# itz-sayak/C-Users-Sayakdutta-Self-Supervised-Arbitrary-Scale-Point-Cloud-Upsampling-via-SNN

Hardware: AMD Instinct MI355X
Metric: upsampled query-points/sec (kNN + fn fwd + rotate + fd fwd + displace), 4x scale, M=48 T=4 (higher is better)
Workload: dtype f32 (GEMMs as 3 x f16 MFMA with f32 accumulation; outer kNN f64); 1 GPU; synthetic sphere N=5000 (seed 0), B=4096 grid queries per GPU per step, M=48, T=4, fn k=[24,18,12] emb 640, fd k=32 scales [8,16,32,48] emb 768, conditioned-random weights seed 0, in-patch kNN recomputed every batch; cloud_points=5000, neighbours=48, outer_knn=f64 brute force, parallelism=query shards x1

## Files before the change

### c-users-sayakdutta-self-supervised-arbitrary-scale-point-cloud-upsampling-via-snn_amd/csrc/fn_edge_chain.hip

```cpp
#include "common.h"
#include "gemm_epi.h"
#include "ops.h"

namespace sapcu {
typedef _Float16 half8 __attribute__((ext_vector_type(8)));

#ifndef SAPCU_CHAIN_LB128
#define SAPCU_CHAIN_LB128 3
#endif
template <int D> struct ChainShape {
    static constexpr int ROWS = D == 128 ? 96 : (D == 256 ? 128 : 64);
    static constexpr int RS = ROWS / 16;
    static constexpr int CB = D == 512 ? 2 : 1;
    static constexpr int CS = 2 * CB;
    static constexpr int NW = D / (32 * CB);
    static constexpr int PLANE = ROWS * 64;
    static constexpr int KSTEP = 2 * PLANE;
    static constexpr int LDS = ROWS * D * 4 + ROWS * 16 + ROWS * 8;
    static constexpr int US = 8;
};

template <int D, int KK> struct ChainSlots {
    static constexpr int GS = 4 * ChainShape<D>::RS;
    static constexpr int SP = GS - KK;
    static constexpr int NUA = (4 * SP) / KK;
    static constexpr int PPG = 4 + NUA;
    static constexpr int point(int rs, int g, int e) {
        const int t = 4 * rs + e;
        if (t < KK) return g;
        const int p = 4 + (g * SP + t - KK) / KK;
        return p < PPG ? p : -1;
    }
    static constexpr int nbr(int rs, int g, int e) {
        const int t = 4 * rs + e;
        return t < KK ? t : (g * SP + t - KK) % KK;
    }
    static constexpr int SP1 = SP > 0 ? SP : 1;
    static constexpr int ua_g(int n, int jj) { return (n * KK + jj) / SP1; }
    static constexpr int ua_rs(int n, int jj) { return (KK + (n * KK + jj) % SP1) >> 2; }
    static constexpr int ua_e(int n, int jj) { return (KK + (n * KK + jj) % SP1) & 3; }
};

__global__ __launch_bounds__(256) void edge_prep_kernel(const float* __restrict__ patch, const int32_t* __restrict__ idx,
                                                        int64_t rows, int m, int kk, int2* __restrict__ tab,
                                                        float4* __restrict__ pd) {
    const int64_t r = (int64_t)blockIdx.x * blockDim.x + threadIdx.x;
    if (r >= rows) return;
    const int64_t pt = r / kk;
    const int64_t nrow = (pt / m) * m + idx[r];
    tab[r] = make_int2((int)pt, (int)nrow);
    const float* pi = patch + pt * 3;
    const float* pj = patch + nrow * 3;
    pd[r] = make_float4(__fsub_rn(pi[0], pj[0]), __fsub_rn(pi[1], pj[1]), __fsub_rn(pi[2], pj[2]), 0.f);
}

__global__ __launch_bounds__(256) void pack_chain_weights_kernel(const _Float16* __restrict__ hi, const _Float16* __restrict__ lo,
                                                                 int d, _Float16* __restrict__ out) {
    const int64_t t = (int64_t)blockIdx.x * blockDim.x + threadIdx.x;
    const int nk32 = d / 32;
    const int64_t total = (int64_t)(d / 16) * nk32 * 2 * 64;
    if (t >= total) return;
    const int lane = (int)(t & 63);
    const int plane = (int)((t >> 6) & 1);
    const int64_t cs_s = t >> 7;
    const int s = (int)(cs_s % nk32), cs = (int)(cs_s / nk32);
    const _Float16* src = (plane ? lo : hi) + (int64_t)(16 * cs + (lane & 15)) * d + 32 * s + 8 * (lane >> 4);
    *reinterpret_cast<half8*>(out + t * 8) = *reinterpret_cast<const half8*>(src);
}

__device__ __forceinline__ float group_bcast(float x, int s) {
    const unsigned a = __float_as_uint(x);
    const auto r = __builtin_amdgcn_permlane16_swap(a, a, false, false);
    const unsigned z = (s & 1) ? r[1] : r[0];
    const auto q = __builtin_amdgcn_permlane32_swap(z, z, false, false);
    return __uint_as_float((s & 2) ? q[1] : q[0]);
}

template <int CS>
struct ChainLane {
    int c16, g;
    int col[CS];
    unsigned xw[CS];
};

template <int CS>
struct ChainW {
    half8 wh[CS], wl[CS];
};

template <int D>
__device__ __forceinline__ half8 chain_w_frag(const half8* __restrict__ wp, int cs, int s, int plane, int lane) {
    return wp[(((int64_t)cs * (D / 32) + s) * 2 + plane) * 64 + lane];
}

template <int D>
__device__ __forceinline__ void chain_w_prefetch(const half8* __restrict__ wp, int cs0, int lane, ChainW<ChainShape<D>::CS>& W) {
#pragma unroll
    for (int j = 0; j < ChainShape<D>::CS; ++j) {
        W.wh[j] = chain_w_frag<D>(wp, cs0 + j, 0, 0, lane);
        W.wl[j] = chain_w_frag<D>(wp, cs0 + j, 0, 1, lane);
    }
}

template <int D>
__device__ __forceinline__ void chain_gemm(const unsigned char* X, const half8* __restrict__ wp, int cs0, int lane,
                                           ChainW<ChainShape<D>::CS>& W, f32x4 (&acc)[ChainShape<D>::RS][ChainShape<D>::CS]) {
    constexpr int NK32 = D / 32, RS = ChainShape<D>::RS, CS = ChainShape<D>::CS, HC = CS / 2;
    constexpr int CH_PLANE = ChainShape<D>::PLANE, CH_KSTEP = ChainShape<D>::KSTEP;
    const int c16 = lane & 15, g = lane >> 4;
    const unsigned char* xa = X + c16 * 64 + ((g ^ ((c16 >> 2) & 3)) * 16);
#pragma unroll
    for (int i = 0; i < RS; ++i)
#pragma unroll
        for (int j = 0; j < CS; ++j) acc[i][j] = f32x4{0.f, 0.f, 0.f, 0.f};
    if (D == 128) {
        constexpr int RH = RS / 2;
#pragma unroll 1
        for (int s = 0; s < NK32; ++s) {
            const int sn = s + 1 < NK32 ? s + 1 : NK32 - 1;
#pragma unroll
            for (int rc = 0; rc < 2; ++rc) {
                half8 ah[RH], al[RH];
#pragma unroll
                for (int i = 0; i < RH; ++i) {
                    ah[i] = *reinterpret_cast<const half8*>(xa + s * CH_KSTEP + (rc * RH + i) * 1024);
                    al[i] = *reinterpret_cast<const half8*>(xa + s * CH_KSTEP + (rc * RH + i) * 1024 + CH_PLANE);
                }
#pragma unroll
                for (int hc = 0; hc < 2; ++hc) {
#pragma unroll
                    for (int i = 0; i < RH; ++i)
#pragma unroll
                        for (int j = hc * HC; j < (hc + 1) * HC; ++j)
                            acc[rc * RH + i][j] = __builtin_amdgcn_mfma_f32_16x16x32_f16(al[i], W.wh[j], acc[rc * RH + i][j], 0, 0, 0);
#pragma unroll
                    for (int i = 0; i < RH; ++i)
#pragma unroll
                        for (int j = hc * HC; j < (hc + 1) * HC; ++j)
                            acc[rc * RH + i][j] = __builtin_amdgcn_mfma_f32_16x16x32_f16(ah[i], W.wl[j], acc[rc * RH + i][j], 0, 0, 0);
#pragma unroll
                    for (int i = 0; i < RH; ++i)
#pragma unroll
                        for (int j = hc * HC; j < (hc + 1) * HC; ++j)
                            acc[rc * RH + i][j] = __builtin_amdgcn_mfma_f32_16x16x32_f16(ah[i], W.wh[j], acc[rc * RH + i][j], 0, 0, 0);
                    if (rc == 1) {
                        __builtin_amdgcn_sched_barrier(0);
#pragma unroll
                        for (int j = hc * HC; j < (hc + 1) * HC; ++j) {
                            W.wh[j] = chain_w_frag<D>(wp, cs0 + j, sn, 0, lane);
                            W.wl[j] = chain_w_frag<D>(wp, cs0 + j, sn, 1, lane);
                        }
                    }
                }
                __builtin_amdgcn_sched_barrier(0);
            }
        }
        return;
    }
#pragma unroll 1
    for (int s = 0; s < NK32; ++s) {
        half8 ah[RS], al[RS];
#pragma unroll
        for (int i = 0; i < RS; ++i) {
            ah[i] = *reinterpret_cast<const half8*>(xa + s * CH_KSTEP + i * 1024);
            al[i] = *reinterpret_cast<const half8*>(xa + s * CH_KSTEP + i * 1024 + CH_PLANE);
        }
        const int sn = s + 1 < NK32 ? s + 1 : NK32 - 1;
#pragma unroll
        for (int hc = 0; hc < 2; ++hc) {
#pragma unroll
            for (int i = 0; i < RS; ++i)
#pragma unroll
                for (int j = hc * HC; j < (hc + 1) * HC; ++j) acc[i][j] = __builtin_amdgcn_mfma_f32_16x16x32_f16(al[i], W.wh[j], acc[i][j], 0, 0, 0);
#pragma unroll
            for (int i = 0; i < RS; ++i)
#pragma unroll
                for (int j = hc * HC; j < (hc + 1) * HC; ++j) acc[i][j] = __builtin_amdgcn_mfma_f32_16x16x32_f16(ah[i], W.wl[j], acc[i][j], 0, 0, 0);
#pragma unroll
            for (int i = 0; i < RS; ++i)
#pragma unroll
                for (int j = hc * HC; j < (hc + 1) * HC; ++j) acc[i][j] = __builtin_amdgcn_mfma_f32_16x16x32_f16(ah[i], W.wh[j], acc[i][j], 0, 0, 0);
            __builtin_amdgcn_sched_barrier(0);
#pragma unroll
            for (int j = hc * HC; j < (hc + 1) * HC; ++j) {
                W.wh[j] = chain_w_frag<D>(wp, cs0 + j, sn, 0, lane);
                W.wl[j] = chain_w_frag<D>(wp, cs0 + j, sn, 1, lane);
            }
        }
    }
}

typedef _Float16 half2v __attribute__((ext_vector_type(2)));
template <int PLANE, int CS>
__device__ __forceinline__ void chain_put2(unsigned char* X, const ChainLane<CS>& L, int cs, int rs, int e, float v0, float v1) {
    unsigned char* p = X + L.xw[cs] + (unsigned)(rs * 1024 + e * 64);
    const f32x2 v = f32x2{v0, v1};
    const half2v hi = __builtin_convertvector(v, half2v);
    half2v lo;
    {
        unsigned lp;
        const unsigned hp = __builtin_bit_cast(unsigned, hi);
        asm volatile("v_fma_mixlo_f16 %0, %1, -1.0, %2 op_sel_hi:[1,0,0]" : "=v"(lp) : "v"(hp), "v"(v.x));
        asm volatile("v_fma_mixhi_f16 %0, %1, -1.0, %2 op_sel:[1,0,0] op_sel_hi:[1,0,0]" : "+v"(lp) : "v"(hp), "v"(v.y));
        lo = __builtin_bit_cast(half2v, lp);
    }
    *reinterpret_cast<_Float16*>(p) = hi.x;
    *reinterpret_cast<_Float16*>(p + 64) = hi.y;
    *reinterpret_cast<_Float16*>(p + PLANE) = lo.x;
    *reinterpret_cast<_Float16*>(p + PLANE + 64) = lo.y;
}

__device__ __forceinline__ void chain_store_split_nt(float* base, int64_t row, int ld, int col, float v) {
    _Float16* rp = reinterpret_cast<_Float16*>(base + row * ld);
    const _Float16 hi = (_Float16)v;
    __builtin_nontemporal_store(hi, &rp[split_hi_index(ld, col)]);
    __builtin_nontemporal_store((_Float16)(v - (float)hi), &rp[split_lo_index(ld, col)]);
}

__device__ __forceinline__ NeuronP chain_lif(const float* __restrict__ lif, int d, int col) {
    NeuronP np;
    np.decay = clampf(lif[col], 0.1f, 0.99f);
    np.adapt = clampf(lif[d + col], 0.001f, 0.1f);
    np.rdecay = clampf(lif[2 * d + col], 0.1f, 0.95f);
    np.theta0 = lif[3 * d + col];
    np.dT = 0.f;
    np.rh = 0.f;
    return np;
}

__device__ __forceinline__ float group_select(float v0, float v1, float v2, float v3, bool g0, bool g1) {
    const float a = g0 ? v1 : v0, b = g0 ? v3 : v2;
    return g1 ? b : a;
}

template <int KK>
__device__ __forceinline__ float chain_softmax_agg(float (&xs)[KK], const float (&ts)[KK]) {
    float mx = -__builtin_huge_valf();
#pragma unroll
    for (int jj = 0; jj < KK; ++jj) mx = fmaxf(mx, xs[jj]);
    float den = 0.f;
    const f32x2 mx2 = f32x2{mx, mx}, l2e = f32x2{1.4426950408889634074f, 1.4426950408889634074f};
#pragma unroll
    for (int jj = 0; jj < KK; jj += 2) {
        const f32x2 e2 = (f32x2{xs[jj], xs[jj + 1]} - mx2) * l2e;
        xs[jj] = __builtin_amdgcn_exp2f(e2.x);
        xs[jj + 1] = __builtin_amdgcn_exp2f(e2.y);
        den = __fadd_rn(den, xs[jj]);
        den = __fadd_rn(den, xs[jj + 1]);
    }
    const float inv_den = __fdiv_rn(1.0f, den);
    const f32x2 inv2 = f32x2{inv_den, inv_den};
    float out = 0.f;
#pragma unroll
    for (int jj = 0; jj < KK; jj += 2) {
        const f32x2 w2 = f32x2{xs[jj], xs[jj + 1]} * inv2;
        out = __fmaf_rn(w2.x, ts[jj], out);
        out = __fmaf_rn(w2.y, ts[jj + 1], out);
    }
    return out;
}

template <int D, int KK, bool O32, bool FILL>
__device__ __forceinline__ void fn_edge_chain_body(const ChainArgs& a) {
    static_assert(!FILL || (D == 512 && KK == 12), "filled groups: d = 512, kk = 12");
    using S = ChainShape<D>;
    using M = ChainSlots<D, KK>;
    constexpr int CH_ROWS = S::ROWS, RS = S::RS, CS = S::CS, CH_PLANE = S::PLANE, CH_KSTEP = S::KSTEP;
    constexpr int PPG = M::PPG, NUA = M::NUA, SP = M::SP;
    constexpr int NUP = RS / 2;
    extern __shared__ __attribute__((aligned(1024))) unsigned char smem[];
    unsigned char* X = smem;
    float* pdx = reinterpret_cast<float*>(smem + CH_ROWS * D * 4);
    float* pdy = pdx + CH_ROWS;
    float* pdz = pdy + CH_ROWS;
    int2* rinfo = reinterpret_cast<int2*>(smem + CH_ROWS * D * 4 + CH_ROWS * 16);

    const int tid = threadIdx.x;
    const int lane = tid & 63;
    const int w = __builtin_amdgcn_readfirstlane(tid >> 6);
    const int cs0 = w * CS;
    ChainLane<CS> L;
    L.c16 = lane & 15;
    L.g = lane >> 4;
    const bool g0 = (L.g & 1) != 0, g1 = (L.g & 2) != 0;
#pragma unroll
    for (int j = 0; j < CS; ++j) {
        L.col[j] = 16 * (cs0 + j) + L.c16;
        L.xw[j] = (unsigned)((L.col[j] >> 5) * CH_KSTEP + L.g * 256 + ((((L.col[j] >> 3) & 3) ^ L.g) * 16) + (L.col[j] & 7) * 2);
    }
    const int rowg = 4 * L.g;

    const int64_t nsuper = FILL ? a.P / 16 : 0;
    const int64_t ngroups = 3 * nsuper + (a.P - 16 * nsuper + PPG - 1) / PPG;
    int64_t grp;
    {
        const int64_t nx = gridDim.x < 8 ? 1 : 8;
        const int64_t x = nx == 1 ? 0 : (blockIdx.x & 7), slot = nx == 1 ? blockIdx.x : (blockIdx.x >> 3);
        const int64_t qd = ngroups / nx, rem = ngroups % nx;
        grp = x * qd + (x < rem ? x : rem) + slot;
        if (slot >= qd + (x < rem ? 1 : 0)) return;
    }
    int64_t pt0 = grp * PPG, strad = -1;
    int spos = 0;
    if (FILL) {
        if (grp < 3 * nsuper) {
            const unsigned sgi = (unsigned)grp / 3u;
            spos = (int)((unsigned)grp - 3u * sgi);
            pt0 = 16 * (int64_t)sgi + PPG * spos;
            strad = 16 * (int64_t)sgi + 15;
        } else {
            pt0 = 16 * nsuper + (grp - 3 * nsuper) * PPG;
        }
    }
    const int npts = (int)((a.P - pt0) < PPG ? (a.P - pt0) : PPG);

    f32x4 acc[RS][CS], pe[RS][CS];
    ChainW<CS> W;
    if (tid < CH_ROWS) {
        const int rs = tid >> 4, sg = (tid >> 2) & 3, e = tid & 3, t = 4 * rs + e;
        int p, jj;
        if (t < KK) {
            p = sg;
            jj = t;
        } else {
            const int u = sg * SP + t - KK;
            p = 4 + u / KK;
            jj = u % KK;
        }
        const bool ok = p < npts;
        int64_t er = ok ? (pt0 + p) * KK + jj : pt0 * KK;
        if (FILL && p >= PPG && strad >= 0) er = strad * KK + 4 * spos + jj;
        const int2 t2 = a.tab[er];
        if (O32) reinterpret_cast<unsigned*>(rinfo)[tid] = (unsigned)t2.y * (unsigned)(a.ldq * 4);
        else rinfo[tid] = t2;
        const float4 dv = a.pd[er];
        pdx[tid] = dv.x;
        pdy[tid] = dv.y;
        pdz[tid] = dv.z;
    }
    lds_barrier();
#pragma unroll
    for (int j = 0; j < CS; ++j) {
        const float wx = a.wd[L.col[j] * 3], wy = a.wd[L.col[j] * 3 + 1], wz = a.wd[L.col[j] * 3 + 2], bd = a.bd[L.col[j]];
        const NeuronP nd = chain_lif(a.lifd, D, L.col[j]);
#pragma unroll
        for (int up = 0; up < NUP; ++up) {
            float v[8];
#pragma unroll
            for (int hq = 0; hq < 2; ++hq) {
                const int r0 = 16 * (2 * up + hq) + rowg;
                const float4 qx = *reinterpret_cast<const float4*>(pdx + r0), qy = *reinterpret_cast<const float4*>(pdy + r0),
                             qz = *reinterpret_cast<const float4*>(pdz + r0);
                const f32x2 wx2 = f32x2{wx, wx}, wy2 = f32x2{wy, wy}, wz2 = f32x2{wz, wz}, bd2 = f32x2{bd, bd};
                const f32x2 ta = pk_fma(wz2, f32x2{qz.x, qz.y}, pk_fma(wy2, f32x2{qy.x, qy.y}, wx2 * f32x2{qx.x, qx.y})) + bd2;
                const f32x2 tb = pk_fma(wz2, f32x2{qz.z, qz.w}, pk_fma(wy2, f32x2{qy.z, qy.w}, wx2 * f32x2{qx.z, qx.w})) + bd2;
                v[4 * hq] = ta.x;
                v[4 * hq + 1] = ta.y;
                v[4 * hq + 2] = tb.x;
                v[4 * hq + 3] = tb.y;
            }
            lif_selfloop_n<8>(v, nd, a.T);
#pragma unroll
            for (int z = 0; z < 8; z += 2) chain_put2<CH_PLANE, CS>(X, L, j, 2 * up + (z >> 2), z & 3, v[z], v[z + 1]);
            __builtin_amdgcn_sched_barrier(0);
        }
    }
    const half8* const wp1 = reinterpret_cast<const half8*>(a.w1p);
    const half8* const wp2 = reinterpret_cast<const half8*>(a.w2p);
    const half8* const wp3 = reinterpret_cast<const half8*>(a.w3p);
    float kq[2][8], vq[2][8];
    auto gather_kv = [&](int j, int up, float (&kd)[8], float (&vd)[8]) {
#pragma unroll
        for (int z = 0; z < 8; ++z) {
            const int row = 16 * (2 * up + (z >> 2)) + rowg + (z & 3);
            if (O32) {
                const unsigned off = reinterpret_cast<const unsigned*>(rinfo)[row] + 4u * (unsigned)L.col[j];
                kd[z] = *reinterpret_cast<const float*>(reinterpret_cast<const char*>(a.qkv + D) + off);
                vd[z] = *reinterpret_cast<const float*>(reinterpret_cast<const char*>(a.qkv + 2 * D) + off);
            } else {
                const int nrow = rinfo[row].y;
                kd[z] = a.qkv[(int64_t)nrow * a.ldq + D + L.col[j]];
                vd[z] = a.qkv[(int64_t)nrow * a.ldq + 2 * D + L.col[j]];
            }
        }
    };
    auto load_q = [&](int j, float& qa, float (&qu)[NUA > 0 ? NUA : 1], float& qs) {
        qa = __builtin_nontemporal_load(&a.qkv[(pt0 + (L.g < npts ? L.g : 0)) * a.ldq + L.col[j]]);
        if (FILL) qs = __builtin_nontemporal_load(&a.qkv[(strad >= 0 ? strad : pt0) * a.ldq + L.col[j]]);
#pragma unroll
        for (int n = 0; n < NUA; ++n) qu[n] = __builtin_nontemporal_load(&a.qkv[(pt0 + (4 + n < npts ? 4 + n : 0)) * a.ldq + L.col[j]]);
    };
    float qa[2], qu[2][NUA > 0 ? NUA : 1], qs[2] = {0.f, 0.f};
    load_q(0, qa[0], qu[0], qs[0]);
    gather_kv(0, 0, kq[0], vq[0]);
    chain_w_prefetch<D>(wp1, cs0, lane, W);
    lds_barrier();

    {
        chain_gemm<D>(X, wp1, cs0, lane, W, acc);
        lds_barrier();
#pragma unroll
        for (int j = 0; j < CS; ++j) {
            const float b1 = a.b1[L.col[j]];
            const NeuronP n1 = chain_lif(a.lif1, D, L.col[j]);
            if (j + 1 < CS) load_q(j + 1, qa[(j + 1) & 1], qu[(j + 1) & 1], qs[(j + 1) & 1]);
#pragma unroll
            for (int up = 0; up < NUP; ++up) {
                const int u = j * NUP + up;
                if (up + 1 < NUP) gather_kv(j, up + 1, kq[(u + 1) & 1], vq[(u + 1) & 1]);
                else if (j + 1 < CS) gather_kv(j + 1, 0, kq[(u + 1) & 1], vq[(u + 1) & 1]);
                __builtin_amdgcn_sched_barrier(0);
                float v[8];
#pragma unroll
                for (int z = 0; z < 8; ++z) v[z] = __fmaf_rn(acc[2 * up + (z >> 2)][j][z & 3], 0.0625f, b1);
                lif_selfloop_n<8>(v, n1, a.T);
                __builtin_amdgcn_sched_barrier(0);
                float ain[8];
#pragma unroll
                for (int z = 0; z < 8; ++z) {
                    const int rs = 2 * up + (z >> 2), e = z & 3;
                    float qv;
                    if (4 * rs + e < KK) {
                        qv = qa[j & 1];
                    } else {
                        float c[4];
#pragma unroll
                        for (int sg = 0; sg < 4; ++sg) {
                            const int p = M::point(rs, sg, e);
                            c[sg] = p >= 4 ? qu[j & 1][p - 4 < NUA ? p - 4 : 0] : (FILL && p < 0 ? qs[j & 1] : qa[j & 1]);
                        }
                        qv = group_select(c[0], c[1], c[2], c[3], g0, g1);
                    }
                    ain[z] = __fadd_rn(__fsub_rn(qv, kq[u & 1][z]), v[z]);
                    pe[rs][j][e] = settle(__fadd_rn(vq[u & 1][z], v[z]));
                }
#pragma unroll
                for (int z = 0; z < 8; z += 2) chain_put2<CH_PLANE, CS>(X, L, j, 2 * up + (z >> 2), z & 3, ain[z], ain[z + 1]);
                __builtin_amdgcn_sched_barrier(0);
            }
        }
        chain_w_prefetch<D>(wp2, cs0, lane, W);
    }
    lds_barrier();
    {
        chain_gemm<D>(X, wp2, cs0, lane, W, acc);
        lds_barrier();
#pragma unroll
        for (int j = 0; j < CS; ++j) {
            const float b2 = a.b2[L.col[j]];
            const NeuronP n2 = chain_lif(a.lif2, D, L.col[j]);
#pragma unroll
            for (int up = 0; up < NUP; ++up) {
                float v[8];
#pragma unroll
                for (int z = 0; z < 8; ++z) v[z] = __fmaf_rn(acc[2 * up + (z >> 2)][j][z & 3], 0.0625f, b2);
                lif_selfloop_n<8>(v, n2, a.T);
#pragma unroll
                for (int z = 0; z < 8; z += 2) chain_put2<CH_PLANE, CS>(X, L, j, 2 * up + (z >> 2), z & 3, v[z], v[z + 1]);
                __builtin_amdgcn_sched_barrier(0);
            }
        }
        chain_w_prefetch<D>(wp3, cs0, lane, W);
    }
    lds_barrier();
    {
        chain_gemm<D>(X, wp3, cs0, lane, W, acc);
#pragma unroll
        for (int j = 0; j < CS; ++j) {
            const float b3 = a.b3[L.col[j]];
#pragma unroll
            for (int i = 0; i < RS; ++i) {
                const f32x2 k16 = f32x2{0.0625f, 0.0625f}, b32 = f32x2{b3, b3}, is2 = f32x2{a.inv_sqrt_hd, a.inv_sqrt_hd};
                const f32x2 lo = pk_fma(f32x2{acc[i][j][0], acc[i][j][1]}, k16, b32) * is2;
                const f32x2 hi = pk_fma(f32x2{acc[i][j][2], acc[i][j][3]}, k16, b32) * is2;
                acc[i][j] = f32x4{lo.x, lo.y, hi.x, hi.y};
            }
            if (FILL) {
                if (L.g == 3 && strad >= 0) {
                    const int64_t o = ((strad >> 4) * KK + 4 * spos) * D + L.col[j];
#pragma unroll
                    for (int e = 0; e < 4; ++e) {
                        __builtin_nontemporal_store(acc[RS - 1][j][e], &a.fill_x[o + e * D]);
                        __builtin_nontemporal_store(pe[RS - 1][j][e], &a.fill_t[o + e * D]);
                    }
                }
            }
            {
                float xs[KK], ts[KK];
#pragma unroll
                for (int jj = 0; jj < KK; ++jj) {
                    xs[jj] = acc[jj >> 2][j][jj & 3];
                    ts[jj] = pe[jj >> 2][j][jj & 3];
                }
                const float out = chain_softmax_agg<KK>(xs, ts);
                if (L.g < npts) {
                    const int64_t pt = pt0 + L.g;
                    if (a.res_split) chain_store_split_nt(a.res, pt, D, L.col[j], out);
                    else __builtin_nontemporal_store(out, &a.res[pt * D + L.col[j]]);
                }
            }
            if (NUA > 0) {
                float xs[KK], ts[KK];
#pragma unroll
                for (int jj = 0; jj < KK; ++jj) {
                    float cx[4] = {0.f, 0.f, 0.f, 0.f}, ct[4] = {0.f, 0.f, 0.f, 0.f};
#pragma unroll
                    for (int n = 0; n < NUA; ++n) {
                        const int rs = M::ua_rs(n, jj), e = M::ua_e(n, jj), sg = M::ua_g(n, jj);
                        cx[n] = group_bcast(acc[rs][j][e], sg);
                        ct[n] = group_bcast(pe[rs][j][e], sg);
                    }
                    xs[jj] = NUA == 1 ? cx[0] : group_select(cx[0], cx[1], cx[2], cx[3], g0, g1);
                    ts[jj] = NUA == 1 ? ct[0] : group_select(ct[0], ct[1], ct[2], ct[3], g0, g1);
                }
                const float out = chain_softmax_agg<KK>(xs, ts);
                if (L.g < NUA && 4 + L.g < npts) {
                    const int64_t pt = pt0 + 4 + L.g;
                    if (a.res_split) chain_store_split_nt(a.res, pt, D, L.col[j], out);
                    else __builtin_nontemporal_store(out, &a.res[pt * D + L.col[j]]);
                }
            }
        }
    }
}

template <int D, int KK, bool O32>
__global__ __launch_bounds__(ChainShape<D>::NW * 64, (D == 128 ? SAPCU_CHAIN_LB128 : 1)) void fn_edge_chain_kernel(const ChainArgs a) {
    fn_edge_chain_body<D, KK, O32, false>(a);
}

template <bool O32>
__global__ __launch_bounds__(ChainShape<512>::NW * 64, 1) void fn_edge_chain_fill_kernel(const ChainArgs a) {
    fn_edge_chain_body<512, 12, O32, true>(a);
}

template <int KK>
__global__ __launch_bounds__(256) void fn_chain_straddler_kernel(const float* __restrict__ fx, const float* __restrict__ ft, int64_t nsuper,
                                                                 int d, float* __restrict__ res, int res_split) {
    const int64_t t = (int64_t)blockIdx.x * blockDim.x + threadIdx.x;
    if (t >= nsuper * d) return;
    const int64_t sgi = t / d;
    const int col = (int)(t - sgi * d);
    float xs[KK], ts[KK];
#pragma unroll
    for (int jj = 0; jj < KK; ++jj) {
        xs[jj] = __builtin_nontemporal_load(&fx[(sgi * KK + jj) * d + col]);
        ts[jj] = __builtin_nontemporal_load(&ft[(sgi * KK + jj) * d + col]);
    }
    const float out = chain_softmax_agg<KK>(xs, ts);
    const int64_t pt = 16 * sgi + 15;
    if (res_split) chain_store_split_nt(res, pt, d, col, out);
    else __builtin_nontemporal_store(out, &res[pt * d + col]);
}

template <int D, int KK, bool O32>
static int launch_chain_t(const ChainArgs& a, hipStream_t st) {
    constexpr int lds = ChainShape<D>::LDS;
    static DeviceOnce lds_once;
    SAPCU_SET_MAX_LDS(lds_once, (&fn_edge_chain_kernel<D, KK, O32>), lds);
    constexpr int PPG = ChainSlots<D, KK>::PPG;
    const int64_t ngroups = (a.P + PPG - 1) / PPG;
    const int64_t grid = ngroups < 8 ? ngroups : ((ngroups + 7) / 8) * 8;
    SAPCU_CHECK_ARG(grid < 0x7fffffffLL, "edge_chain: too many groups");
    hipLaunchKernelGGL((fn_edge_chain_kernel<D, KK, O32>), dim3((unsigned)grid), dim3(ChainShape<D>::NW * 64), lds, st, a);
    SAPCU_CHECK_LAUNCH();
    return SAPCU_OK;
}

template <bool O32>
static int launch_chain_fill_t(const ChainArgs& a, hipStream_t st) {
    constexpr int lds = ChainShape<512>::LDS, PPG = ChainSlots<512, 12>::PPG;
    static DeviceOnce lds_once;
    SAPCU_SET_MAX_LDS(lds_once, (&fn_edge_chain_fill_kernel<O32>), lds);
    const int64_t nsuper = a.P / 16;
    const int64_t ngroups = 3 * nsuper + (a.P - 16 * nsuper + PPG - 1) / PPG;
    const int64_t grid = ngroups < 8 ? ngroups : ((ngroups + 7) / 8) * 8;
    SAPCU_CHECK_ARG(grid < 0x7fffffffLL, "edge_chain: too many groups");
    hipLaunchKernelGGL((fn_edge_chain_fill_kernel<O32>), dim3((unsigned)grid), dim3(ChainShape<512>::NW * 64), lds, st, a);
    SAPCU_CHECK_LAUNCH();
    hipLaunchKernelGGL((fn_chain_straddler_kernel<12>), dim3((unsigned)((nsuper * 512 + 255) / 256)), dim3(256), 0, st, a.fill_x, a.fill_t,
                       nsuper, 512, a.res, a.res_split);
    SAPCU_CHECK_LAUNCH();
    return SAPCU_OK;
}

bool fn_edge_chain_ok(int d, int kk) { return (d == 128 && kk == 24) || (d == 256 && kk == 18) || (d == 512 && kk == 12); }

int launch_fn_edge_chain(ChainArgs a, const float* patch, const int32_t* idx, int d, int kk, int2* tab, float4* pd,
                         hipStream_t st) {
    if (a.P == 0) return SAPCU_OK;
    SAPCU_CHECK_ARG(fn_edge_chain_ok(d, kk), "edge_chain: unsupported block shape d=%d kk=%d", d, kk);
    SAPCU_CHECK_ARG(a.P * (int64_t)kk < 0x7fffffffLL && a.P * (int64_t)(a.ldq) < (1LL << 40), "edge_chain: too many rows");
    const int64_t rows = a.P * kk;
    hipLaunchKernelGGL(edge_prep_kernel, dim3((unsigned)((rows + 255) / 256)), dim3(256), 0, st, patch, idx, rows, a.m, kk, tab, pd);
    SAPCU_CHECK_LAUNCH();
    a.tab = tab;
    a.pd = pd;
    const bool o32 = !a.wide_offsets && (uint64_t)a.P * (uint64_t)a.ldq * 4u + 3u * (uint64_t)d * 4u < (1ull << 32) && a.ldq > 0;
    if (d == 128) return o32 ? launch_chain_t<128, 24, true>(a, st) : launch_chain_t<128, 24, false>(a, st);
    if (d == 256) return o32 ? launch_chain_t<256, 18, true>(a, st) : launch_chain_t<256, 18, false>(a, st);
    if (a.fill_x && a.fill_t && a.P >= 16) return o32 ? launch_chain_fill_t<true>(a, st) : launch_chain_fill_t<false>(a, st);
    return o32 ? launch_chain_t<512, 12, true>(a, st) : launch_chain_t<512, 12, false>(a, st);
}

int launch_pack_chain_weights(const void* w16_hi, const void* w16_lo, int d, void* out, hipStream_t st) {
    const int64_t total = (int64_t)(d / 16) * (d / 32) * 2 * 64;
    hipLaunchKernelGGL(pack_chain_weights_kernel, dim3((unsigned)((total + 255) / 256)), dim3(256), 0, st,
                       (const _Float16*)w16_hi, (const _Float16*)w16_lo, d, (_Float16*)out);
    SAPCU_CHECK_LAUNCH();
    return SAPCU_OK;
}

}
```

### c-users-sayakdutta-self-supervised-arbitrary-scale-point-cloud-upsampling-via-snn_amd/csrc/model.hip

```cpp
#include <stdarg.h>
#include <stdlib.h>

#include <new>
#include <vector>

#include "common.h"
#include "ops.h"

namespace sapcu {

static thread_local char g_err[512] = "";

void set_error(const char* fmt, ...) {
    va_list ap;
    va_start(ap, fmt);
    vsnprintf(g_err, sizeof(g_err), fmt, ap);
    va_end(ap);
}

enum FnSlot {
    FN_STEM_W = 0, FN_STEM_B, FN_STEM_LIF,
    FN_BLK0 = 3,
    FN_FINAL_W = FN_BLK0 + 63, FN_FINAL_B, FN_FINAL_LIF,
    FN_FCOUT_W, FN_FCOUT_B,
    FN_MLP0_W, FN_MLP0_B, FN_MLP1_W, FN_MLP1_B, FN_MLP2_W, FN_MLP2_B,
    FN_HEAD_W, FN_HEAD_B, FN_LN_W, FN_LN_B,
    FN_SLOTS
};
enum FnBlkSlot {
    B_FC1_W = 0, B_FC1_B, B_SNN1,
    B_QKV_W, B_QKV_B, B_QKV_LIF,
    B_DELTA_W, B_DELTA_B, B_DELTA_LIF,
    B_DELTA2_W, B_DELTA2_B, B_DELTA2_LIF,
    B_GAMMA_W, B_GAMMA_B, B_GAMMA_LIF,
    B_GAMMA2_W, B_GAMMA2_B,
    B_OUT_W, B_OUT_B,
    B_FC2_W, B_FC2_B,
    B_SLOTS
};
static_assert(B_SLOTS == 21, "fn block slot count");
static_assert(FN_SLOTS == 81, "fn slot count");

enum FdSlot {
    FD_E0_W = 0, FD_E0_B,
    FD_FUSE_W, FD_FUSE_B, FD_SNN0,
    FD_EDGE1_W, FD_EDGE1_SHIFT, FD_SNN1,
    FD_EDGE2_W, FD_EDGE2_SHIFT, FD_SNN2,
    FD_EDGE3_W, FD_EDGE3_SHIFT, FD_SNN3,
    FD_MSC_W, FD_MSC_B,
    FD_TI_W, FD_SNNFC,
    FD_FCIN_W, FD_FCIN_B,
    FD_R0_FC0_W, FD_R0_FC0_B, FD_R0_FC4_W, FD_R0_FC4_B, FD_R0_PROJ_W, FD_R0_PROJ_B,
    FD_R1_FC0_W, FD_R1_FC0_B, FD_R1_FC4_W, FD_R1_FC4_B, FD_R1_PROJ_W, FD_R1_PROJ_B,
    FD_QKV_W, FD_QKV_B,
    FD_WO_T, FD_BO, FD_LN_W, FD_LN_B, FD_WH_T, FD_BH, FD_WD, FD_BD,
    FD_SLOTS
};
static_assert(FD_SLOTS == 42, "fd slot count");

}

struct sapcu_model {
    int kind = 0;
    int kv[3] = {0, 0, 0};
    int k = 0, nscale = 0;
    int ks[8] = {0, 0, 0, 0, 0, 0, 0, 0};
    int32_t* ks_dev = nullptr;
    int* gate_dev = nullptr;
    bool sf16 = true;
    void* w16_hi = nullptr;
    void* w16_lo = nullptr;
    void* chain_w = nullptr;
    int* ovf_dev = nullptr;
    int emb = 0, T = 0, heads = 0;
    int64_t chunk = 0;
    int64_t ws_budget = 0;
    bool opt_bt = true;
    bool opt_chain = true;
    bool opt_chain_wide = false;
    bool opt_chain_fill = true;
    bool opt_shortk = true;
    bool opt_fn_maxfuse = true;
    bool opt_fn_fold_out = true;
    bool opt_fd_maxfuse = true;
    bool opt_fd_split = true;
    bool opt_fd_fused = true;
    bool opt_fd_x0 = true;
    void* fde_w = nullptr;
    int64_t fde_off[5] = {0, 0, 0, 0, 0};
    float* fde_nprm = nullptr;
    float* blob = nullptr;
    int64_t blob_floats = 0;
    int64_t fold_w[3] = {0, 0, 0}, fold_b[3] = {0, 0, 0};
    std::vector<int64_t> dir;
    const float* p(int slot) const { return blob + dir[slot]; }
};

namespace sapcu {

static inline int64_t imax(int64_t a, int64_t b) { return a > b ? a : b; }
static inline int imin(int a, int b) { return a < b ? a : b; }

static bool split_rows_gemm_on_big_tile(const GemmArgs& g, bool allow_bt) { return allow_bt && gemm_sf16_bt_ok(g); }

int launch_gemm_split_rows(const GemmArgs& g, hipStream_t st, bool allow_bt) {
    if (split_rows_gemm_on_big_tile(g, allow_bt)) return launch_gemm_sf16_bt(g, st);
    return launch_gemm_sf16_ring(g, st);
}

static void fold_affine_f64(const float* w1, const float* b1, const float* w2, const float* b2, int d, int n, float* w_fold,
                            float* b_fold) {
    std::vector<double> acc((size_t)d);
    for (int i = 0; i < n; ++i) {
        for (int k = 0; k < d; ++k) acc[k] = 0.0;
        double bs = 0.0;
        for (int j = 0; j < d; ++j) {
            const double a = (double)w2[(int64_t)i * d + j];
            const float* row = w1 + (int64_t)j * d;
            for (int k = 0; k < d; ++k) acc[k] += a * (double)row[k];
            bs += a * (double)b1[j];
        }
        for (int k = 0; k < d; ++k) w_fold[(int64_t)i * d + k] = (float)acc[k];
        b_fold[i] = (float)(bs + (double)b2[i]);
    }
}

static bool env_is(const char* name, const char* value) {
    const char* e = getenv(name);
    return e && strcmp(e, value) == 0;
}

static void read_env_switches(sapcu_model* m) {
    m->sf16 = !env_is("SAPCU_GEMM", "f32");
    m->opt_bt = !env_is("SAPCU_BT", "0");
    m->opt_chain = !env_is("SAPCU_CHAIN", "0");
    m->opt_chain_wide = env_is("SAPCU_CHAIN", "wide");
    m->opt_chain_fill = !env_is("SAPCU_CHAIN_FILL", "0");
    m->opt_shortk = !env_is("SAPCU_SHORTK", "0");
    m->opt_fn_maxfuse = !env_is("SAPCU_FN_MAXFUSE", "0");
    m->opt_fn_fold_out = !env_is("SAPCU_FN_FOLD_OUT", "0");
    m->opt_fd_maxfuse = !env_is("SAPCU_FD_MAXFUSE", "0");
    m->opt_fd_split = !env_is("SAPCU_FD_SPLIT", "0");
    m->opt_fd_fused = !env_is("SAPCU_FD_FUSED", "0");
    m->opt_fd_x0 = !env_is("SAPCU_FD_X0", "0");
    const char* ce = getenv("SAPCU_CHUNK");
    m->chunk = ce ? atoll(ce) : 0;
    if (m->chunk < 0) m->chunk = 0;
    const char* be = getenv("SAPCU_WS_BUDGET_MB");
    m->ws_budget = (be ? atoll(be) : 20480) * (int64_t)(1 << 20);
    if (m->ws_budget < (int64_t)(64 << 20)) m->ws_budget = (int64_t)(64 << 20);
}

static void free_model(sapcu_model* m) {
    void* const owned[] = {m->w16_hi, m->w16_lo, m->chain_w, m->ovf_dev, m->blob, m->ks_dev, m->gate_dev, m->fde_w, m->fde_nprm};
    for (void* p : owned)
        if (p) (void)hipFree(p);
    delete m;
}

static int run_gemm(const sapcu_model* m, GemmArgs& g, hipStream_t st) {
    const bool have16 = m && m->sf16 && g.w >= m->blob && g.w < m->blob + m->blob_floats;
    if (have16) {
        const int64_t off = g.w - m->blob;
        g.w16_hi = (const _Float16*)m->w16_hi + off;
        g.w16_lo = (const _Float16*)m->w16_lo + off;
        g.ovf = m->ovf_dev;
        if (g.a_split) return launch_gemm_split_rows(g, st, m->opt_bt);
        if (m->opt_shortk && gemm_shortk_ok(g)) return launch_gemm_shortk(g, st);
        if (g.max_out) {
            set_error("run_gemm: a direct max output needs the short-K kernel");
            return SAPCU_ERR_ARG;
        }
        if (g.k % 64 == 0) return launch_gemm_sf16(g, st);
    }
    if (g.a_split || g.c_split || g.c2_split) {
        set_error("run_gemm: split-row operands need the split-f16 kernels");
        return SAPCU_ERR_ARG;
    }
    return launch_gemm(g, st);
}

static int gemm(const sapcu_model* m, const float* a, int64_t r, int k, int lda, const float* w, int n,
                const float* bias, float* c, int ldc, int epi, hipStream_t st, const float* lif = nullptr,
                int lifT = 0, const float* resid = nullptr, int ldr = 0, int fmt = 0) {
    GemmArgs g;
    memset(&g, 0, sizeof(g));
    g.a = a; g.r = r; g.k = k; g.lda = lda; g.w = w; g.n = n; g.bias = bias; g.c = c; g.ldc = ldc;
    g.epi = epi; g.lif = lif; g.lif_T = lifT; g.resid = resid; g.ldr = ldr;
    g.a_split = fmt & 1; g.c_split = (fmt >> 1) & 1;
    return run_gemm(m, g, st);
}

#define SAPCU_TRY(expr)                 \
    do {                                \
        int _rc = (expr);               \
        if (_rc != SAPCU_OK) return _rc; \
    } while (0)

static int tap_copy(void* const* taps, int which, int64_t dst_off_bytes, const void* src, int64_t bytes,
                    hipStream_t st) {
    if (!taps || !taps[which] || bytes == 0) return SAPCU_OK;
    SAPCU_CHECK_HIP(hipMemcpyAsync((char*)taps[which] + dst_off_bytes, src, (size_t)bytes, hipMemcpyDeviceToDevice, st));
    return SAPCU_OK;
}

struct FnPlan {
    int64_t cb;
    int kk[3], kmx;
    int64_t edge_floats, edge_floats23;
};

static bool fn_block_fused(const sapcu_model* m, int l, int mp) {
    return m->sf16 && m->chain_w && m->opt_chain && fn_edge_chain_ok(128 << l, imin(m->kv[l], mp));
}

static int fn_kmax(const sapcu_model* m, int mp) {
    int kmx = 1;
    for (int l = 0; l < 3; ++l) kmx = kmx > imin(m->kv[l], mp) ? kmx : imin(m->kv[l], mp);
    return kmx;
}

static void fn_edge_floats_per_patch(const sapcu_model* m, int mp, int64_t& first, int64_t& others) {
    first = (int64_t)mp * m->emb;
    others = 0;
    for (int l = 0; l < 3; ++l) {
        if (fn_block_fused(m, l, mp)) continue;
        const int64_t e = (int64_t)mp * imin(m->kv[l], mp) * (128 << l);
        first = imax(first, e);
        others = imax(others, e);
    }
}

static int64_t fn_bytes_per_patch(const sapcu_model* m, int mp) {
    int64_t e1, e23;
    fn_edge_floats_per_patch(m, mp, e1, e23);
    int64_t idxs = 0;
    for (int l = 0; l < 3; ++l) idxs += (int64_t)mp * imin(m->kv[l], mp) * 4;
    return (e1 + 2 * e23) * 4 + idxs + (int64_t)mp * fn_kmax(m, mp) * 24 + (int64_t)mp * (64 + 192 + 512 + 1536 + 512) * 4 +
           ((int64_t)m->emb + 2048 + 1024 + 512 + 256 + 3) * 4;
}

static int64_t chunk_patches(const sapcu_model* m, int64_t b, int64_t bytes_per_patch) {
    int64_t cb = m->chunk;
    if (cb <= 0) {
        cb = m->ws_budget / (bytes_per_patch > 0 ? bytes_per_patch : 1);
        cb = cb < 64 ? 64 : (cb / 64) * 64;
    }
    if (cb > b) cb = b;
    return cb < 1 ? 1 : cb;
}

static FnPlan fn_plan(const sapcu_model* m, int64_t b, int mp) {
    FnPlan pl;
    pl.cb = chunk_patches(m, b, fn_bytes_per_patch(m, mp));
    for (int l = 0; l < 3; ++l) pl.kk[l] = imin(m->kv[l], mp);
    pl.kmx = fn_kmax(m, mp);
    int64_t e1, e23;
    fn_edge_floats_per_patch(m, mp, e1, e23);
    pl.edge_floats = e1 * pl.cb;
    pl.edge_floats23 = e23 * pl.cb;
    return pl;
}

struct FnWs {
    int32_t* idx[3];
    int2* tab;
    float4* pdiff;
    float *feat0, *cat, *X, *QKV, *RES;
    float* B1;
    float *B2, *B3;
    float *pooled, *enc, *h1, *h2, *h3, *logits;
    size_t bytes;
};

static FnWs fn_ws_layout(void* base, const sapcu_model* m, const FnPlan& pl, int mp) {
    const int64_t P = pl.cb * mp;
    WsCarver c(base);
    FnWs w;
    for (int l = 0; l < 3; ++l) w.idx[l] = c.take<int32_t>(P * pl.kk[l]);
    w.tab = c.take<int2>(P * pl.kmx);
    w.pdiff = c.take<float4>(P * pl.kmx);
    w.feat0 = c.take<float>(P * 64);
    w.cat = c.take<float>(P * 192);
    w.X = c.take<float>(P * 512);
    w.QKV = c.take<float>(P * 1536);
    w.RES = c.take<float>(P * 512);
    w.B1 = c.take<float>(pl.edge_floats);
    w.B2 = c.take<float>(pl.edge_floats23);
    w.B3 = c.take<float>(pl.edge_floats23);
    w.pooled = c.take<float>(pl.cb * m->emb);
    w.enc = c.take<float>(pl.cb * 2048);
    w.h1 = c.take<float>(pl.cb * 1024);
    w.h2 = c.take<float>(pl.cb * 512);
    w.h3 = c.take<float>(pl.cb * 256);
    w.logits = c.take<float>(pl.cb * 3);
    w.bytes = c.bytes();
    return w;
}

static int64_t chain_w_off(int l, int q) {
    int64_t off = 0;
    for (int i = 0; i < l; ++i) off += (int64_t)3 * 2 * (128 << i) * (128 << i);
    return off + (int64_t)q * 2 * (128 << l) * (128 << l);
}

struct FnEdge {
    const float* pc;
    int64_t P;
    int mp, l, d, kk, sb, SP;
    float sqrt_hd;
    int64_t b1_floats;
};

static int fn_edge_chain_fused(const sapcu_model* m, const FnWs& W, const FnEdge& e, hipStream_t st) {
    const int d = e.d, sb = e.sb;
    ChainArgs ca;
    memset(&ca, 0, sizeof(ca));
    ca.P = e.P; ca.m = e.mp; ca.qkv = W.QKV; ca.ldq = 3 * d;
    ca.wd = m->p(sb + B_DELTA_W); ca.bd = m->p(sb + B_DELTA_B); ca.lifd = m->p(sb + B_DELTA_LIF);
    const _Float16* cw = (const _Float16*)m->chain_w;
    ca.w1p = cw + chain_w_off(e.l, 0); ca.b1 = m->p(sb + B_DELTA2_B); ca.lif1 = m->p(sb + B_DELTA2_LIF);
    ca.w2p = cw + chain_w_off(e.l, 1); ca.b2 = m->p(sb + B_GAMMA_B); ca.lif2 = m->p(sb + B_GAMMA_LIF);
    ca.w3p = cw + chain_w_off(e.l, 2); ca.b3 = m->p(sb + B_GAMMA2_B);
    ca.inv_sqrt_hd = 1.0f / e.sqrt_hd;
    ca.res = W.RES; ca.res_split = e.SP; ca.T = 4; ca.wide_offsets = m->opt_chain_wide ? 1 : 0;
    if (m->opt_chain_fill && d == 512 && e.kk == 12) {
        const int64_t need = (e.P / 16) * 12 * 512;
        if (need > 0 && need <= e.P * 512 && need <= e.b1_floats) {
            ca.fill_x = W.X;
            ca.fill_t = W.B1;
        }
    }
    return launch_fn_edge_chain(ca, e.pc, W.idx[e.l], d, e.kk, W.tab, W.pdiff, st);
}

static int fn_edge_chain_unfused(const sapcu_model* m, const FnWs& W, const FnEdge& e, hipStream_t st) {
    const int d = e.d, kk = e.kk, sb = e.sb, SP = e.SP;
    const int64_t R = e.P * kk;
    const int32_t* idx = W.idx[e.l];
    SAPCU_TRY(launch_fn_pe1(e.pc, idx, R, e.mp, kk, d, m->p(sb + B_DELTA_W), m->p(sb + B_DELTA_B), m->p(sb + B_DELTA_LIF), 4, W.B1, SP,
                            st));
    {
        GemmArgs g;
        memset(&g, 0, sizeof(g));
        g.a = W.B1; g.r = R; g.k = d; g.lda = d; g.w = m->p(sb + B_DELTA2_W); g.n = d;
        g.bias = m->p(sb + B_DELTA2_B); g.c = W.B2; g.ldc = d; g.epi = EPI_LIF_ATTN;
        g.lif = m->p(sb + B_DELTA2_LIF); g.lif_T = 4; g.c2 = W.B3;
        g.q = W.QKV; g.kf = W.QKV + d; g.ldq = 3 * d; g.tab = W.tab;
        g.a_split = SP; g.c2_split = SP;
        SAPCU_TRY(launch_edge_table(idx, R, e.mp, kk, W.tab, st));
        SAPCU_TRY(run_gemm(m, g, st));
    }
    SAPCU_TRY(gemm(m, W.B3, R, d, d, m->p(sb + B_GAMMA_W), d, m->p(sb + B_GAMMA_B), W.B1, d, EPI_LIF, st, m->p(sb + B_GAMMA_LIF), 4,
                   nullptr, 0, SP | (SP << 1)));
    SAPCU_TRY(gemm(m, W.B1, R, d, d, m->p(sb + B_GAMMA2_W), d, m->p(sb + B_GAMMA2_B), W.B3, d, EPI_BIAS, st, nullptr, 0, nullptr, 0, SP));
    return launch_fn_softmax_agg(W.B3, W.B2, W.QKV + 2 * d, 3 * d, idx, e.P, e.mp, kk, d, e.sqrt_hd, W.RES, SP, st);
}

static int fn_forward(const sapcu_model* m, const float* patch, int64_t b, int mp, const int32_t* knn_in,
                      int32_t* knn_out, float* normals, void* ws, int64_t ws_bytes, void* const* taps,
                      hipStream_t st) {
    const FnPlan pl = fn_plan(m, b, mp);
    const FnWs W = fn_ws_layout(ws_align256(ws), m, pl, mp);
    if (ws_bytes < (int64_t)W.bytes + 256) {
        set_error("fn_forward: workspace %lld B < required %lld B", (long long)ws_bytes, (long long)W.bytes + 256);
        return SAPCU_ERR_WORKSPACE;
    }
    int64_t tab_off[3];
    tab_off[0] = 0;
    tab_off[1] = b * mp * pl.kk[0];
    tab_off[2] = tab_off[1] + b * mp * pl.kk[1];

    for (int64_t s = 0; s < b; s += pl.cb) {
        const int64_t cb = (b - s) < pl.cb ? (b - s) : pl.cb;
        const int64_t P = cb * mp;
        const float* pc = patch + s * mp * 3;

        if (!knn_in) SAPCU_TRY(launch_patch_knn_multi(pc, cb, (int64_t)mp * 3, mp, 3, 3, 3, pl.kk, W.idx, st));
        for (int l = 0; l < 3; ++l) {
            const int64_t cnt = P * pl.kk[l];
            if (knn_in)
                SAPCU_CHECK_HIP(hipMemcpyAsync(W.idx[l], knn_in + tab_off[l] + s * mp * pl.kk[l], cnt * 4,
                                               hipMemcpyDeviceToDevice, st));
            if (knn_out)
                SAPCU_CHECK_HIP(hipMemcpyAsync(knn_out + tab_off[l] + s * mp * pl.kk[l], W.idx[l], cnt * 4,
                                               hipMemcpyDeviceToDevice, st));
        }
        SAPCU_TRY(launch_fn_stem(pc, P, m->p(FN_STEM_W), m->p(FN_STEM_B), m->p(FN_STEM_LIF), m->T, W.feat0, st));
        SAPCU_TRY(tap_copy(taps, SAPCU_FN_TAP_STEM, s * mp * 64 * 4, W.feat0, P * 64 * 4, st));

        const float* fin = W.feat0;
        int ldin = 64;
        for (int l = 0; l < 3; ++l) {
            const int d = 128 << l;
            const int sb = FN_BLK0 + l * B_SLOTS;
            const int SP = m->sf16 ? 1 : 0;
            float* const out = W.cat + 64 * l;
            SAPCU_TRY(gemm(m, fin, P, 64, ldin, m->p(sb + B_FC1_W), d, m->p(sb + B_FC1_B), W.X, d, EPI_LIF, st,
                           m->p(sb + B_SNN1), 4, nullptr, 0, SP << 1));
            SAPCU_TRY(gemm(m, W.X, P, d, d, m->p(sb + B_QKV_W), 3 * d, m->p(sb + B_QKV_B), W.QKV, 3 * d, EPI_LIF, st,
                           m->p(sb + B_QKV_LIF), 4, nullptr, 0, SP));
            const FnEdge e{pc, P, mp, l, d, pl.kk[l], sb, SP, (float)sqrt((double)(d / m->heads)), pl.edge_floats};
            SAPCU_TRY(fn_block_fused(m, l, mp) ? fn_edge_chain_fused(m, W, e, st) : fn_edge_chain_unfused(m, W, e, st));
            if (m->opt_fn_fold_out) {
                SAPCU_TRY(gemm(m, W.RES, P, d, d, m->blob + m->fold_w[l], 64, m->blob + m->fold_b[l], out, 192, EPI_RESID, st,
                               nullptr, 0, fin, ldin, SP));
            } else {
                SAPCU_TRY(gemm(m, W.RES, P, d, d, m->p(sb + B_OUT_W), d, m->p(sb + B_OUT_B), W.X, d, EPI_BIAS, st, nullptr, 0, nullptr,
                               0, SP | (SP << 1)));
                SAPCU_TRY(gemm(m, W.X, P, d, d, m->p(sb + B_FC2_W), 64, m->p(sb + B_FC2_B), out, 192, EPI_RESID, st,
                               nullptr, 0, fin, ldin, SP));
            }
            if (taps && taps[SAPCU_FN_TAP_BLOCK1 + l]) {
                SAPCU_CHECK_HIP(hipMemcpy2DAsync((char*)taps[SAPCU_FN_TAP_BLOCK1 + l] + s * mp * 64 * 4, 64 * 4,
                                                 out, 192 * 4, 64 * 4, (size_t)P, hipMemcpyDeviceToDevice, st));
            }
            fin = out;
            ldin = 192;
        }
        if (m->sf16 && m->opt_fn_maxfuse) {
            GemmArgs g;
            memset(&g, 0, sizeof(g));
            g.a = W.cat; g.r = P; g.k = 192; g.lda = 192; g.w = m->p(FN_FINAL_W); g.n = m->emb; g.bias = m->p(FN_FINAL_B);
            g.ldc = m->emb; g.epi = EPI_LIF_MAX; g.lif = m->p(FN_FINAL_LIF); g.lif_T = m->T;
            g.max_keys = reinterpret_cast<unsigned*>(W.B1); g.max_m = mp;
            const bool direct = m->opt_shortk && mp == 48;
            if (direct) g.max_out = W.pooled;
            else SAPCU_CHECK_HIP(hipMemsetAsync(g.max_keys, 0, (size_t)cb * m->emb * 4, st));
            SAPCU_TRY(run_gemm(m, g, st));
            if (!direct) SAPCU_TRY(launch_decode_max_keys(g.max_keys, cb * m->emb, W.pooled, st));
        } else {
            SAPCU_TRY(gemm(m, W.cat, P, 192, 192, m->p(FN_FINAL_W), m->emb, m->p(FN_FINAL_B), W.B1, m->emb, EPI_LIF, st,
                           m->p(FN_FINAL_LIF), m->T));
            SAPCU_TRY(launch_rowgroup_max(W.B1, cb, mp, m->emb, W.pooled, st));
        }
        SAPCU_TRY(tap_copy(taps, SAPCU_FN_TAP_POOLED, s * m->emb * 4, W.pooled, cb * m->emb * 4, st));
        SAPCU_TRY(gemm(m, W.pooled, cb, m->emb, m->emb, m->p(FN_FCOUT_W), 2048, m->p(FN_FCOUT_B), W.enc, 2048, EPI_BIAS, st));
        SAPCU_TRY(tap_copy(taps, SAPCU_FN_TAP_ENC, s * 2048 * 4, W.enc, cb * 2048 * 4, st));
        SAPCU_TRY(gemm(m, W.enc, cb, 2048, 2048, m->p(FN_MLP0_W), 1024, m->p(FN_MLP0_B), W.h1, 1024, EPI_GELU, st));
        SAPCU_TRY(gemm(m, W.h1, cb, 1024, 1024, m->p(FN_MLP1_W), 512, m->p(FN_MLP1_B), W.h2, 512, EPI_GELU, st));
        SAPCU_TRY(gemm(m, W.h2, cb, 512, 512, m->p(FN_MLP2_W), 256, m->p(FN_MLP2_B), W.h3, 256, EPI_GELU, st));
        SAPCU_TRY(launch_fn_tail(W.h3, cb, 256, m->p(FN_HEAD_W), m->p(FN_HEAD_B), m->p(FN_LN_W), m->p(FN_LN_B), W.logits,
                                 normals + s * 3, st));
        SAPCU_TRY(tap_copy(taps, SAPCU_FN_TAP_LOGITS, s * 3 * 4, W.logits, cb * 3 * 4, st));
    }
    return SAPCU_OK;
}

struct FdPlan {
    int64_t cb;
    int kmax0, kk;
    bool fused;
    bool x0path;
    bool maxfuse;
    int64_t agg_rows(int mp) const { return maxfuse ? 1 : mp; }
};

static bool fd_encoder_fused(const sapcu_model* m, int mp) {
    return m->sf16 && m->opt_fd_fused && m->fde_w && m->fde_nprm && fd_encoder_ok(mp, m->nscale, m->emb, m->T);
}

static bool fd_x0_path(const sapcu_model* m, int mp) {
    return !fd_encoder_fused(m, mp) && m->sf16 && m->opt_fd_fused && m->opt_fd_x0 && m->opt_fd_maxfuse && m->opt_fd_split && m->fde_w &&
           m->fde_nprm && fd_msc_ok(mp, m->emb, m->T);
}

static int fd_kmax0(const sapcu_model* m, int mp) {
    int kmax = 1;
    for (int i = 0; i < m->nscale; ++i) kmax = kmax > m->ks[i] ? kmax : m->ks[i];
    return imin(kmax, mp);
}

static FdPlan fd_plan(const sapcu_model* m, int64_t b, int mp) {
    FdPlan pl;
    pl.fused = fd_encoder_fused(m, mp);
    pl.x0path = fd_x0_path(m, mp);
    pl.maxfuse = m->sf16 && m->opt_fd_maxfuse;
    pl.kmax0 = fd_kmax0(m, mp);
    pl.kk = imin(m->k, mp);
    int64_t per_patch = ((int64_t)(m->T + 1) * m->emb + 256 + 3 * 128 + 3 * 64 + 192 + 64) * 4;
    if (!pl.fused) {
        const int64_t slabs = pl.x0path ? 2 : m->T;
        per_patch = (int64_t)mp * ((slabs * 960 + 960 + 1024 + 64 * (m->nscale + 1)) * 4 + (int64_t)(pl.kmax0 + 3 * pl.kk) * 4) +
                    (int64_t)m->T * pl.agg_rows(mp) * m->emb * 4 + per_patch;
    }
    pl.cb = chunk_patches(m, b, per_patch);
    return pl;
}

struct FdWs {
    int32_t* idx0;
    int32_t* idxb;
    float* E0;
    float* FUSED;
    float* SPK;
    float* F0;
    float* AB;
    float* AGG;
    float* X0;
    float *POOLED, *ENC;
    float *D1, *D2a, *D2b, *D2c, *D3a, *D3b, *D3c, *QKV, *ATT;
    size_t bytes;
};

static FdWs fd_ws_layout(void* base, const sapcu_model* m, const FdPlan& pl, int mp) {
    const int64_t cb = pl.cb, T = m->T, emb = m->emb;
    const int64_t P = pl.fused ? 0 : cb * mp;
    WsCarver c(base);
    FdWs w;
    w.idx0 = c.take<int32_t>(P * pl.kmax0);
    w.idxb = c.take<int32_t>(3 * P * pl.kk);
    w.E0 = c.take<float>(P * 64 * m->nscale);
    w.FUSED = c.take<float>(P * 64);
    w.SPK = c.take<float>((pl.x0path ? 1 : T) * P * 960);
    w.F0 = c.take<float>(P * 960);
    w.AB = c.take<float>(P * 1024);
    w.AGG = c.take<float>(pl.fused ? 0 : T * cb * pl.agg_rows(mp) * emb);
    w.X0 = c.take<float>(pl.x0path ? P * 960 : 0);
    w.POOLED = c.take<float>(T * cb * emb);
    w.ENC = c.take<float>(cb * emb);
    w.D1 = c.take<float>(cb * 256);
    w.D2a = c.take<float>(cb * 128);
    w.D2b = c.take<float>(cb * 128);
    w.D2c = c.take<float>(cb * 128);
    w.D3a = c.take<float>(cb * 64);
    w.D3b = c.take<float>(cb * 64);
    w.D3c = c.take<float>(cb * 64);
    w.QKV = c.take<float>(cb * 192);
    w.ATT = c.take<float>(cb * 64);
    w.bytes = c.bytes();
    return w;
}

struct FdChunk {
    const float* pc;
    int64_t s, cb, b;
    int mp;
    const int32_t* knn_force;
    void* const* taps;
    int64_t P() const { return cb * mp; }
    float* tap(int which) const { return taps ? (float*)taps[which] : nullptr; }
    float* x0_tap() const { return tap(SAPCU_FD_TAP_X0) ? tap(SAPCU_FD_TAP_X0) + s * mp * 960 : nullptr; }
};

static const int FD_CIN[4] = {0, 64, 128, 256}, FD_COUT[4] = {64, 128, 256, 512}, FD_COFF[4] = {0, 64, 192, 448};

static int fd_encode_fused(const sapcu_model* m, const FdPlan& pl, const FdWs& W, const FdChunk& c, hipStream_t st) {
    FdEncArgs ea;
    memset(&ea, 0, sizeof(ea));
    ea.patch = c.pc; ea.b = c.cb; ea.b_total = c.b; ea.s0 = c.s;
    ea.m = c.mp; ea.T = m->T; ea.kk = pl.kk; ea.kmax0 = pl.kmax0; ea.nscale = m->nscale; ea.emb = m->emb;
    for (int i = 0; i < 4; ++i) ea.ks[i] = i < m->nscale ? imin(m->ks[i], c.mp) : 0;
    ea.e0_w = m->p(FD_E0_W); ea.e0_b = m->p(FD_E0_B);
    const _Float16* fw = (const _Float16*)m->fde_w;
    ea.fuse_wp = fw + m->fde_off[0]; ea.fuse_b = m->p(FD_FUSE_B);
    for (int l = 0; l < 3; ++l) {
        ea.edge_wp[l] = fw + m->fde_off[1 + l];
        ea.shift[l] = m->p(FD_EDGE1_SHIFT + 3 * l);
    }
    ea.msc_wp = fw + m->fde_off[4]; ea.msc_b = m->p(FD_MSC_B);
    ea.nprm = m->fde_nprm;
    ea.pooled = W.POOLED;
    ea.knn_force = c.knn_force;
    ea.tap_knn = (int32_t*)c.tap(SAPCU_FD_TAP_KNN);
    ea.tap_fused0 = c.tap(SAPCU_FD_TAP_FUSED0);
    ea.tap_spikes = c.tap(SAPCU_FD_TAP_SPIKES);
    ea.tap_x0 = c.tap(SAPCU_FD_TAP_X0);
    ea.gate = m->gate_dev; ea.ovf = m->ovf_dev;
    return launch_fd_encoder(ea, st);
}

static GemmArgs fd_msc_gemm_args(const sapcu_model* m, const FdWs& W, const FdChunk& c) {
    GemmArgs mg;
    memset(&mg, 0, sizeof(mg));
    mg.a = W.SPK; mg.r = (int64_t)m->T * c.P(); mg.k = 960; mg.lda = 960; mg.w = m->p(FD_MSC_W); mg.n = m->emb; mg.bias = m->p(FD_MSC_B);
    mg.c = nullptr; mg.ldc = m->emb; mg.epi = EPI_LRELU_MAX; mg.max_keys = reinterpret_cast<unsigned*>(W.AGG); mg.max_m = c.mp;
    return mg;
}

static int fd_front(const sapcu_model* m, const FdPlan& pl, const FdWs& W, const FdChunk& c, bool& split_spikes, hipStream_t st) {
    const int T = m->T, mp = c.mp;
    const int64_t P = c.P(), cb = c.cb, s = c.s, b = c.b;
    void* const* taps = c.taps;
    SAPCU_TRY(launch_patch_knn(c.pc, cb, mp, 3, 3, pl.kmax0, W.idx0, st));
    SAPCU_TRY(launch_fd_edge0(c.pc, W.idx0, pl.kmax0, P, mp, m->nscale, m->ks_dev, m->p(FD_E0_W), m->p(FD_E0_B), W.E0, st));
    SAPCU_TRY(gemm(m, W.E0, P, 64 * m->nscale, 64 * m->nscale, m->p(FD_FUSE_W), 64, m->p(FD_FUSE_B), W.FUSED, 64, EPI_LRELU, st));
    SAPCU_TRY(tap_copy(taps, SAPCU_FD_TAP_FUSED0, s * mp * 64 * 4, W.FUSED, P * 64 * 4, st));
    float* const X0T = c.x0_tap();
    if (X0T) SAPCU_CHECK_HIP(hipMemcpy2DAsync(X0T, 960 * 4, W.FUSED, 64 * 4, 64 * 4, (size_t)P, hipMemcpyDeviceToDevice, st));
    split_spikes = pl.x0path;
    if (!pl.x0path && pl.maxfuse && m->opt_fd_split && !c.tap(SAPCU_FD_TAP_SPIKES)) {
        GemmArgs probe = fd_msc_gemm_args(m, W, c);
        probe.a_split = 1;
        probe.w16_hi = (const _Float16*)m->w16_hi + (probe.w - m->blob);
        probe.w16_lo = (const _Float16*)m->w16_lo + (probe.w - m->blob);
        split_spikes = split_rows_gemm_on_big_tile(probe, m->opt_bt);
    }
    float* const SPKS = split_spikes ? W.SPK : nullptr;
    float* const SPK0 = split_spikes ? W.F0 : W.SPK;
    float* const X0P = pl.x0path ? W.X0 : nullptr;
    SAPCU_TRY(launch_fd_neuron(true, 0, W.FUSED, 64, nullptr, 0, mp, nullptr, P, 64, m->p(FD_SNN0), T, SPK0, 960, 0,
                               nullptr, m->gate_dev, st, SPKS, X0P));
    for (int l = 1; l <= 3; ++l) {
        const int cin = FD_CIN[l], cout = FD_COUT[l], coff = FD_COFF[l - 1];
        int32_t* idl = W.idxb + (int64_t)(l - 1) * pl.cb * mp * pl.kk;
        const float* F = SPK0 + coff;
        if (c.knn_force) {
            SAPCU_CHECK_HIP(hipMemcpyAsync(idl, c.knn_force + ((int64_t)(l - 1) * b + s) * mp * pl.kk, P * pl.kk * 4,
                                           hipMemcpyDeviceToDevice, st));
        } else {
            SAPCU_TRY(launch_patch_knn_strided(F, cb, (int64_t)mp * 960, mp, cin, 960, pl.kk, idl, st));
        }
        if (c.tap(SAPCU_FD_TAP_KNN))
            SAPCU_CHECK_HIP(hipMemcpyAsync((int32_t*)taps[SAPCU_FD_TAP_KNN] + ((int64_t)(l - 1) * b + s) * mp * pl.kk,
                                           idl, P * pl.kk * 4, hipMemcpyDeviceToDevice, st));
        const int ew = FD_EDGE1_W + 3 * (l - 1);
        if (split_spikes)
            SAPCU_TRY(gemm(m, SPKS + coff, P, cin, 960, m->p(ew), 2 * cout, nullptr, W.AB, 2 * cout, EPI_BIAS, st, nullptr, 0, nullptr, 0,
                           1));
        else
            SAPCU_TRY(gemm(m, F, P, cin, 960, m->p(ew), 2 * cout, nullptr, W.AB, 2 * cout, EPI_BIAS, st));
        SAPCU_TRY(launch_fd_neuron(l == 1, 1, W.AB, 2 * cout, idl, pl.kk, mp, m->p(ew + 1), P, cout, m->p(ew + 2), T, SPK0, 960,
                                   FD_COFF[l], nullptr, m->gate_dev, st, SPKS, X0P));
        if (X0T && !pl.x0path)
            SAPCU_TRY(launch_fd_pre(W.AB, 2 * cout, idl, pl.kk, mp, m->p(ew + 1), P, cout, X0T, 960, FD_COFF[l], st));
    }
    return SAPCU_OK;
}

static int fd_msc_from_x0(const sapcu_model* m, const FdWs& W, const FdChunk& c, hipStream_t st) {
    if (c.x0_tap()) SAPCU_CHECK_HIP(hipMemcpyAsync(c.x0_tap(), W.X0, (size_t)c.P() * 960 * 4, hipMemcpyDeviceToDevice, st));
    FdMscArgs ma;
    memset(&ma, 0, sizeof(ma));
    ma.x0 = W.X0; ma.b = c.cb; ma.b_total = c.b; ma.s0 = c.s; ma.m = c.mp; ma.T = m->T; ma.emb = m->emb;
    ma.msc_wp = (const _Float16*)m->fde_w + m->fde_off[4]; ma.msc_b = m->p(FD_MSC_B); ma.nprm = m->fde_nprm;
    ma.pooled = W.POOLED; ma.tap_spikes = c.tap(SAPCU_FD_TAP_SPIKES); ma.gate = m->gate_dev;
    return launch_fd_msc(ma, st);
}

static int fd_msc_from_slabs(const sapcu_model* m, const FdPlan& pl, const FdWs& W, const FdChunk& c, bool split_spikes, hipStream_t st) {
    const int T = m->T, emb = m->emb;
    const int64_t P = c.P();
    if (c.tap(SAPCU_FD_TAP_SPIKES)) {
        for (int t = 0; t < T; ++t)
            SAPCU_CHECK_HIP(hipMemcpyAsync(c.tap(SAPCU_FD_TAP_SPIKES) + ((int64_t)t * c.b + c.s) * c.mp * 960,
                                           W.SPK + (int64_t)t * P * 960, P * 960 * 4, hipMemcpyDeviceToDevice, st));
    }
    if (pl.maxfuse) {
        GemmArgs mg = fd_msc_gemm_args(m, W, c);
        SAPCU_CHECK_HIP(hipMemsetAsync(mg.max_keys, 0, (size_t)T * c.cb * emb * 4, st));
        mg.a_split = split_spikes ? 1 : 0;
        SAPCU_TRY(run_gemm(m, mg, st));
        return launch_decode_max_keys(mg.max_keys, (int64_t)T * c.cb * emb, W.POOLED, st);
    }
    SAPCU_TRY(gemm(m, W.SPK, (int64_t)T * P, 960, 960, m->p(FD_MSC_W), emb, m->p(FD_MSC_B), W.AGG, emb, EPI_LRELU, st));
    return launch_rowgroup_max(W.AGG, (int64_t)T * c.cb, c.mp, emb, W.POOLED, st);
}

static int fd_temporal_decoder(const sapcu_model* m, const FdWs& W, const FdChunk& c, float* dist, hipStream_t st) {
    const int T = m->T, emb = m->emb;
    const int64_t cb = c.cb, s = c.s;
    if (c.tap(SAPCU_FD_TAP_POOLED)) {
        for (int t = 0; t < T; ++t)
            SAPCU_CHECK_HIP(hipMemcpyAsync(c.tap(SAPCU_FD_TAP_POOLED) + ((int64_t)t * c.b + s) * emb, W.POOLED + (int64_t)t * cb * emb,
                                           cb * emb * 4, hipMemcpyDeviceToDevice, st));
    }
    SAPCU_TRY(launch_fd_temporal(W.POOLED, T, cb, emb, m->p(FD_TI_W), m->p(FD_SNNFC), W.ENC, st));
    SAPCU_TRY(tap_copy(c.taps, SAPCU_FD_TAP_ENC, s * emb * 4, W.ENC, cb * emb * 4, st));
    SAPCU_TRY(gemm(m, W.ENC, cb, emb, emb, m->p(FD_FCIN_W), 256, m->p(FD_FCIN_B), W.D1, 256, EPI_GELU, st));
    SAPCU_TRY(gemm(m, W.D1, cb, 256, 256, m->p(FD_R0_FC0_W), 128, m->p(FD_R0_FC0_B), W.D2a, 128, EPI_GELU, st));
    SAPCU_TRY(gemm(m, W.D1, cb, 256, 256, m->p(FD_R0_PROJ_W), 128, m->p(FD_R0_PROJ_B), W.D2b, 128, EPI_BIAS, st));
    SAPCU_TRY(gemm(m, W.D2a, cb, 128, 128, m->p(FD_R0_FC4_W), 128, m->p(FD_R0_FC4_B), W.D2c, 128, EPI_RESID_GELU, st, nullptr, 0, W.D2b,
                   128));
    SAPCU_TRY(gemm(m, W.D2c, cb, 128, 128, m->p(FD_R1_FC0_W), 64, m->p(FD_R1_FC0_B), W.D3a, 64, EPI_GELU, st));
    SAPCU_TRY(gemm(m, W.D2c, cb, 128, 128, m->p(FD_R1_PROJ_W), 64, m->p(FD_R1_PROJ_B), W.D3b, 64, EPI_BIAS, st));
    SAPCU_TRY(gemm(m, W.D3a, cb, 64, 64, m->p(FD_R1_FC4_W), 64, m->p(FD_R1_FC4_B), W.D3c, 64, EPI_RESID_GELU, st, nullptr, 0, W.D3b, 64));
    SAPCU_TRY(gemm(m, W.D3c, cb, 64, 64, m->p(FD_QKV_W), 192, m->p(FD_QKV_B), W.QKV, 192, EPI_BIAS, st));
    return launch_fd_tail(W.D3c, W.QKV, cb, m->heads, m->p(FD_WO_T), m->p(FD_BO), m->p(FD_LN_W), m->p(FD_LN_B), m->p(FD_WH_T),
                          m->p(FD_BH), m->p(FD_WD), m->p(FD_BD), W.ATT, dist + s, st);
}

static int fd_forward(const sapcu_model* m, const float* patch, int64_t b, int mp, const int32_t* knn_force,
                      float* dist, void* ws, int64_t ws_bytes, void* const* taps, hipStream_t st) {
    const FdPlan pl = fd_plan(m, b, mp);
    const FdWs W = fd_ws_layout(ws_align256(ws), m, pl, mp);
    if (ws_bytes < (int64_t)W.bytes + 256) {
        set_error("fd_forward: workspace %lld B < required %lld B", (long long)ws_bytes, (long long)W.bytes + 256);
        return SAPCU_ERR_WORKSPACE;
    }
    for (int64_t s = 0; s < b; s += pl.cb) {
        const FdChunk c{patch + s * mp * 3, s, (b - s) < pl.cb ? (b - s) : pl.cb, b, mp, knn_force, taps};
        if (pl.fused) {
            SAPCU_TRY(fd_encode_fused(m, pl, W, c, st));
        } else {
            bool split_spikes = false;
            SAPCU_TRY(fd_front(m, pl, W, c, split_spikes, st));
            SAPCU_TRY(pl.x0path ? fd_msc_from_x0(m, W, c, st) : fd_msc_from_slabs(m, pl, W, c, split_spikes, st));
        }
        SAPCU_TRY(fd_temporal_decoder(m, W, c, dist, st));
    }
    return SAPCU_OK;
}

}

using namespace sapcu;

extern "C" {

int sapcu_abi_version(void) { return SAPCU_ABI_VERSION; }
const char* sapcu_last_error(void) { return g_err; }

int sapcu_knn_gather_f64(const double* cloud, int64_t n, const double* queries, int64_t b, int k, int64_t* idx_out,
                         double* dist_out, float* patch_out, void* stream) {
    SAPCU_CHECK_ARG(cloud && queries && idx_out, "knn_gather: null pointer");
    SAPCU_CHECK_ARG(n >= 1 && b >= 0 && k >= 1 && k <= 128 && k <= n, "knn_gather: need 1 <= k <= min(128, n) (n=%lld k=%d)",
                    (long long)n, k);
    SAPCU_CHECK_ARG(n < 0x7fffffffLL, "knn_gather: n too large");
    return launch_knn_outer(cloud, n, queries, b, k, idx_out, dist_out, patch_out, (hipStream_t)stream);
}

int sapcu_gather_rotate_f64(const double* cloud, int64_t n, const double* queries, int64_t b, const int64_t* idx, int k,
                            const float* normals, float* patch_out, void* stream) {
    SAPCU_CHECK_ARG(cloud && queries && idx && patch_out, "gather_rotate: null pointer");
    SAPCU_CHECK_ARG(n >= 1 && b >= 0 && k >= 1, "gather_rotate: bad sizes");
    return launch_gather_rotate(cloud, n, queries, b, idx, k, normals, patch_out, (hipStream_t)stream);
}

int sapcu_displace_f64(const double* queries, const float* normals, const float* dist, int64_t b, double* out,
                       void* stream) {
    SAPCU_CHECK_ARG(queries && normals && dist && out && b >= 0, "displace: bad argument");
    return launch_displace(queries, normals, dist, b, out, (hipStream_t)stream);
}

int64_t sapcu_fps_workspace_bytes(int64_t npoint) { return npoint < 0 ? -1 : (int64_t)fps_workspace_bytes((int)npoint); }

int sapcu_fps_f32(const float* xyz, int64_t n, int64_t npoint, int64_t* idx_out, void* workspace, int64_t workspace_bytes,
                  void* stream) {
    SAPCU_CHECK_ARG(npoint >= 0 && npoint <= n && n < (int64_t)1 << 31, "fps: need 0 <= npoint <= n < 2^31 (n=%lld npoint=%lld)",
                    (long long)n, (long long)npoint);
    if (npoint == 0) return SAPCU_OK;
    SAPCU_CHECK_ARG(xyz && idx_out && workspace, "fps: null pointer");
    SAPCU_CHECK_ARG(((uintptr_t)workspace & 7) == 0, "fps: the workspace must be 8-byte aligned (64-bit mailboxes)");
    if (workspace_bytes < (int64_t)fps_workspace_bytes((int)npoint)) {
        set_error("fps: workspace of %lld bytes, need %lld", (long long)workspace_bytes,
                  (long long)fps_workspace_bytes((int)npoint));
        return SAPCU_ERR_WORKSPACE;
    }
    int rc = launch_fps(xyz, n, (int)npoint, (int)(n / 2), idx_out, workspace, (hipStream_t)stream);
    if (rc != SAPCU_OK) return rc;
    SAPCU_CHECK_HIP(hipStreamSynchronize((hipStream_t)stream));
    int flag = 0;
    rc = fps_failed(workspace, (int)npoint, &flag);
    if (rc != SAPCU_OK) return rc;
    if (flag) {
        set_error("fps: a workgroup of the persistent grid never arrived at the step barrier (grid not resident)");
        return SAPCU_ERR_HIP;
    }
    return SAPCU_OK;
}

int sapcu_neuron_selfloop(const float* x, int64_t rows, int channels, int steps, const float* membrane_decay,
                          const float* threshold_adapt, const float* refractory_decay, const float* threshold_base,
                          const float* delta_T, const float* theta_rh, float* spikes_out, float* membrane_out,
                          float* threshold_out, float* refractory_out, void* stream) {
    SAPCU_CHECK_ARG(x && membrane_decay && threshold_adapt && refractory_decay && threshold_base, "neuron: null pointer");
    SAPCU_CHECK_ARG((delta_T == nullptr) == (theta_rh == nullptr), "neuron: delta_T and theta_rh go together");
    SAPCU_CHECK_ARG(rows >= 0 && channels >= 1 && steps >= 1, "neuron: bad sizes");
    return launch_neuron_selfloop(x, rows, channels, steps, membrane_decay, threshold_adapt, refractory_decay,
                                  threshold_base, delta_T, theta_rh, spikes_out, membrane_out, threshold_out,
                                  refractory_out, (hipStream_t)stream);
}

int sapcu_neuron_drive(const float* x, int64_t rows, int channels, int steps, const float* membrane_decay,
                       const float* threshold_adapt, const float* refractory_decay, const float* threshold_base,
                       const float* delta_T, const float* theta_rh, int channel_pairs, float* spikes_out, float* membrane_out,
                       float* threshold_out, float* refractory_out, int* gate_open_out, void* stream) {
    SAPCU_CHECK_ARG(x && membrane_decay && threshold_adapt && refractory_decay && threshold_base, "neuron_drive: null pointer");
    SAPCU_CHECK_ARG((delta_T == nullptr) == (theta_rh == nullptr), "neuron_drive: delta_T and theta_rh go together");
    SAPCU_CHECK_ARG(rows >= 0 && channels >= 1 && steps >= 1, "neuron_drive: bad sizes");
    return launch_neuron_drive(x, rows, channels, steps, membrane_decay, threshold_adapt, refractory_decay, threshold_base, delta_T,
                               theta_rh, channel_pairs, spikes_out, membrane_out, threshold_out, refractory_out, gate_open_out,
                               (hipStream_t)stream);
}

int sapcu_patch_knn(const float* feat, int64_t b, int m, int c, int ld, int k, int32_t* idx_out, void* stream) {
    SAPCU_CHECK_ARG(feat && idx_out && b >= 0 && ld >= c, "patch_knn: bad argument");
    return launch_patch_knn(feat, b, m, c, ld, k, idx_out, (hipStream_t)stream);
}

int sapcu_l2_normalize3(const float* in, float* out, int64_t b, void* stream) {
    SAPCU_CHECK_ARG(in && out && b >= 0, "l2_normalize3: bad argument");
    return launch_l2_normalize3(in, out, b, (hipStream_t)stream);
}

static int split_into_ws(const float* w, int64_t cnt, void* w16_ws, GemmArgs& g, hipStream_t st) {
    char* base = (char*)w16_ws;
    int* ovf = (int*)(base + 4 * cnt);
    SAPCU_CHECK_HIP(hipMemsetAsync(ovf, 0, sizeof(int), st));
    SAPCU_TRY(launch_split_weights(w, cnt, base, base + 2 * cnt, ovf, st));
    g.w16_hi = (const _Float16*)base;
    g.w16_lo = (const _Float16*)(base + 2 * cnt);
    g.ovf = ovf;
    return SAPCU_OK;
}

int sapcu_gemm_f32(const float* a, int64_t r, int k, int lda, const float* w, int n, const float* bias,
                   const float* lif4, int lif_steps, float* c, int ldc, void* w16_ws, int a_split_rows, int c_split_rows,
                   void* stream) {
    SAPCU_CHECK_ARG(a && w && c && r >= 0 && n >= 1, "gemm: bad argument");
    SAPCU_CHECK_ARG(!lif4 || lif_steps >= 1, "gemm: lif_steps must be >= 1");
    SAPCU_CHECK_ARG(!(a_split_rows || c_split_rows) || w16_ws, "gemm: split rows need the split-f16 kernels (w16_ws)");
    SAPCU_CHECK_ARG(r == 0 || (k > 0 && k % 32 == 0 && lda >= k && ldc >= n), "gemm: need k %% 32 == 0, lda >= k and ldc >= n (k=%d lda=%d n=%d ldc=%d)", k, lda, n, ldc);
    SAPCU_CHECK_ARG(r == 0 || ((((uintptr_t)a | (uintptr_t)w | (uintptr_t)w16_ws) & 15) == 0 && lda % (a_split_rows ? 8 : 4) == 0),
                    "gemm: A, W and w16_ws must be 16-byte aligned, lda %% 4 == 0 (%% 8 for split rows) (lda=%d)", lda);
    GemmArgs g;
    memset(&g, 0, sizeof(g));
    g.a = a; g.r = r; g.k = k; g.lda = lda; g.w = w; g.n = n; g.bias = bias; g.c = c; g.ldc = ldc;
    g.epi = lif4 ? EPI_LIF : EPI_BIAS; g.lif = lif4; g.lif_T = lif_steps;
    g.a_split = a_split_rows ? 1 : 0; g.c_split = c_split_rows ? 1 : 0;
    if (w16_ws && (g.a_split || k % 64 == 0)) {
        SAPCU_TRY(split_into_ws(w, (int64_t)n * k, w16_ws, g, (hipStream_t)stream));
        if (g.a_split) return launch_gemm_split_rows(g, (hipStream_t)stream, a_split_rows != 2);
        if (!env_is("SAPCU_SHORTK", "0") && gemm_shortk_ok(g)) return launch_gemm_shortk(g, (hipStream_t)stream);
        return launch_gemm_sf16(g, (hipStream_t)stream);
    }
    SAPCU_CHECK_ARG(!g.c_split, "gemm: split-row output needs k %% 64 == 0 on the f32-A path");
    return launch_gemm(g, (hipStream_t)stream);
}

int sapcu_to_split_rows(const float* in, int64_t rows, int k, int ld_in, float* out, int ld_out, void* stream) {
    SAPCU_CHECK_ARG(in && out && rows >= 0 && k >= 1 && ld_in >= k && ld_out >= k, "to_split_rows: bad argument");
    return launch_to_split_rows(in, rows, k, ld_in, out, ld_out, (hipStream_t)stream);
}

int sapcu_posenc_gemm_f32(const float* pe1, int64_t r, int d, const float* w, const float* bias, const float* lif4,
                          int lif_steps, const float* qkv, const int32_t* idx, int kk, int m_pts, float* pe_out,
                          float* attn_in_out, void* edge_table_ws, void* w16_ws, int split_rows, void* stream) {
    SAPCU_CHECK_ARG(pe1 && w && lif4 && qkv && idx && pe_out && attn_in_out && edge_table_ws && r >= 0 && d >= 32 &&
                        lif_steps >= 1 && kk >= 1 && m_pts >= 1,
                    "posenc_gemm: bad argument");
    SAPCU_CHECK_ARG(!split_rows || w16_ws, "posenc_gemm: split rows need the split-f16 kernels (w16_ws)");
    SAPCU_CHECK_ARG(d % 32 == 0, "posenc_gemm: d=%d must be a multiple of 32", d);
    SAPCU_CHECK_ARG((((uintptr_t)pe1 | (uintptr_t)w | (uintptr_t)w16_ws) & 15) == 0 && ((uintptr_t)edge_table_ws & 7) == 0,
                    "posenc_gemm: pe1, w and w16_ws must be 16-byte aligned, edge_table_ws 8-byte aligned");
    GemmArgs g;
    memset(&g, 0, sizeof(g));
    g.a = pe1; g.r = r; g.k = d; g.lda = d; g.w = w; g.n = d; g.bias = bias; g.c = pe_out; g.ldc = d;
    g.epi = EPI_LIF_ATTN; g.lif = lif4; g.lif_T = lif_steps; g.c2 = attn_in_out;
    g.q = qkv; g.kf = qkv + d; g.ldq = 3 * d; g.tab = (const int2*)edge_table_ws;
    SAPCU_TRY(launch_edge_table(idx, r, m_pts, kk, (int2*)edge_table_ws, (hipStream_t)stream));
    if (w16_ws && (split_rows || d % 64 == 0)) {
        SAPCU_TRY(split_into_ws(w, (int64_t)d * d, w16_ws, g, (hipStream_t)stream));
        if (split_rows) {
            g.a_split = 1;
            g.c2_split = 1;
            return launch_gemm_split_rows(g, (hipStream_t)stream, split_rows != 2);
        }
        return launch_gemm_sf16(g, (hipStream_t)stream);
    }
    return launch_gemm(g, (hipStream_t)stream);
}

struct ChainWs {
    int2* tab;
    float4* pd;
    char* split[3];
    _Float16* packed[3];
    size_t bytes;
};

static ChainWs chain_ws_layout(void* base, int64_t points, int d, int kk) {
    WsCarver c(base);
    ChainWs w;
    w.tab = c.take<int2>(points * kk);
    w.pd = c.take<float4>(points * kk);
    for (int q = 0; q < 3; ++q) {
        w.split[q] = c.take<char>((int64_t)d * d * 4 + 16);
        w.packed[q] = c.take<_Float16>((int64_t)d * d * 2);
    }
    w.bytes = c.bytes();
    return w;
}

int64_t sapcu_fn_edge_chain_workspace_bytes(int64_t points, int d, int kk) {
    if (points < 0 || !fn_edge_chain_ok(d, kk)) {
        set_error("fn_edge_chain_workspace_bytes: unsupported shape (d=%d kk=%d)", d, kk);
        return SAPCU_ERR_ARG;
    }
    return (int64_t)chain_ws_layout(nullptr, points, d, kk).bytes + 256;
}

int sapcu_fn_edge_chain_f32(const float* patch, const int32_t* idx, int64_t points, int m_pts, int d, int kk,
                            const float* qkv, const float* w_delta, const float* b_delta, const float* lif_delta,
                            const float* w1, const float* b1, const float* lif1, const float* w2, const float* b2,
                            const float* lif2, const float* w3, const float* b3, int heads, int lif_steps,
                            float* res_out, void* workspace, int64_t workspace_bytes, void* stream) {
    SAPCU_CHECK_ARG(patch && idx && qkv && w_delta && b_delta && lif_delta && w1 && b1 && lif1 && w2 && b2 && lif2 && w3 && b3 &&
                        res_out && workspace, "fn_edge_chain: null pointer");
    SAPCU_CHECK_ARG(fn_edge_chain_ok(d, kk), "fn_edge_chain: unsupported shape (d=%d kk=%d)", d, kk);
    SAPCU_CHECK_ARG(points >= 0 && m_pts >= kk && heads >= 1 && d % heads == 0 && lif_steps >= 1, "fn_edge_chain: bad sizes");
    const int64_t need = sapcu_fn_edge_chain_workspace_bytes(points, d, kk);
    if (workspace_bytes < need) {
        set_error("fn_edge_chain: workspace %lld B < required %lld B", (long long)workspace_bytes, (long long)need);
        return SAPCU_ERR_WORKSPACE;
    }
    hipStream_t st = (hipStream_t)stream;
    const ChainWs W = chain_ws_layout(ws_align256(workspace), points, d, kk);
    const float* ws[3] = {w1, w2, w3};
    for (int q = 0; q < 3; ++q) {
        GemmArgs g;
        memset(&g, 0, sizeof(g));
        SAPCU_TRY(split_into_ws(ws[q], (int64_t)d * d, W.split[q], g, st));
        SAPCU_TRY(launch_pack_chain_weights(g.w16_hi, g.w16_lo, d, W.packed[q], st));
    }
    ChainArgs ca;
    memset(&ca, 0, sizeof(ca));
    ca.P = points; ca.m = m_pts; ca.qkv = qkv; ca.ldq = 3 * d;
    ca.wd = w_delta; ca.bd = b_delta; ca.lifd = lif_delta;
    ca.w1p = W.packed[0]; ca.b1 = b1; ca.lif1 = lif1;
    ca.w2p = W.packed[1]; ca.b2 = b2; ca.lif2 = lif2;
    ca.w3p = W.packed[2]; ca.b3 = b3;
    ca.inv_sqrt_hd = 1.0f / (float)sqrt((double)(d / heads));
    ca.res = res_out; ca.res_split = 0; ca.T = lif_steps;
    return launch_fn_edge_chain(ca, patch, idx, d, kk, W.tab, W.pd, st);
}

int sapcu_model_create(int kind, const int32_t* hp, int n_hp, const float* blob, int64_t blob_floats,
                       const int64_t* dir_host, int n_dir, sapcu_model_t* out) {
    SAPCU_CHECK_ARG(hp && blob && dir_host && out && blob_floats > 0, "model_create: null pointer");
    sapcu_model* m = new (std::nothrow) sapcu_model();
    SAPCU_CHECK_ARG(m != nullptr, "model_create: out of host memory");
    m->kind = kind;
    read_env_switches(m);
    int rc = SAPCU_OK;
    if (kind == SAPCU_KIND_FN) {
        if (n_hp != 6 || n_dir != FN_SLOTS) {
            set_error("model_create(fn): need 6 hparams and %d slots (got %d, %d)", (int)FN_SLOTS, n_hp, n_dir);
            rc = SAPCU_ERR_ARG;
        } else {
            m->kv[0] = hp[0]; m->kv[1] = hp[1]; m->kv[2] = hp[2];
            m->emb = hp[3]; m->T = hp[4]; m->heads = hp[5];
            if (m->kv[0] < 1 || m->kv[1] < 1 || m->kv[2] < 1 || m->emb < 32 || m->emb % 32 || m->T < 1 || m->heads < 1 ||
                128 % m->heads) {
                set_error("model_create(fn): unsupported hyper-parameters");
                rc = SAPCU_ERR_ARG;
            }
        }
    } else if (kind == SAPCU_KIND_FD) {
        if (n_hp < 6 || n_dir != FD_SLOTS || hp[4] < 1 || hp[4] > 8 || n_hp != 5 + hp[4]) {
            set_error("model_create(fd): need [k,emb,T,heads,S,ks...] and %d slots", (int)FD_SLOTS);
            rc = SAPCU_ERR_ARG;
        } else {
            m->k = hp[0]; m->emb = hp[1]; m->T = hp[2]; m->heads = hp[3]; m->nscale = hp[4];
            for (int i = 0; i < m->nscale; ++i) m->ks[i] = hp[5 + i];
            if (m->k < 1 || m->emb < 32 || m->emb % 32 || m->T < 1 || m->T > 64) {
                set_error("model_create(fd): unsupported hyper-parameters");
                rc = SAPCU_ERR_ARG;
            } else if (m->heads < 1 || m->heads > 64 || (m->heads & (m->heads - 1))) {
                set_error("model_create(fd): num_heads must be a power of two <= 64 (got %d)", m->heads);
                rc = SAPCU_ERR_ARG;
            }
            for (int i = 0; i < m->nscale && rc == SAPCU_OK; ++i)
                if (m->ks[i] < 1) {
                    set_error("model_create(fd): k_scales[%d] = %d, need >= 1", i, m->ks[i]);
                    rc = SAPCU_ERR_ARG;
                }
        }
    } else {
        set_error("model_create: unknown kind %d", kind);
        rc = SAPCU_ERR_ARG;
    }
    if (rc == SAPCU_OK) {
        m->dir.assign(dir_host, dir_host + n_dir);
        for (int i = 0; i < n_dir; ++i)
            if (m->dir[i] < 0 || m->dir[i] >= blob_floats || (m->dir[i] & 3)) {
                set_error("model_create: slot %d offset %lld out of range / unaligned", i, (long long)m->dir[i]);
                rc = SAPCU_ERR_ARG;
                break;
            }
    }
    auto hip_ok = [&](hipError_t e, const char* what) {
        if (e != hipSuccess && rc == SAPCU_OK) {
            set_error("model_create: %s failed: %s", what, hipGetErrorString(e));
            rc = SAPCU_ERR_HIP;
        }
    };
    if (rc == SAPCU_OK) {
        int64_t total = blob_floats;
        if (kind == SAPCU_KIND_FN && m->opt_fn_fold_out) {
            total = (total + 63) & ~(int64_t)63;
            for (int l = 0; l < 3; ++l) {
                m->fold_w[l] = total;
                total += (int64_t)64 * (128 << l);
                m->fold_b[l] = total;
                total += 64;
            }
        }
        m->blob_floats = total;
        hip_ok(hipMalloc((void**)&m->blob, (size_t)total * 4), "hipMalloc(blob)");
        if (rc == SAPCU_OK) hip_ok(hipMemcpy(m->blob, blob, (size_t)blob_floats * 4, hipMemcpyDeviceToDevice), "copy blob");
        if (rc == SAPCU_OK && total > blob_floats)
            hip_ok(hipMemset(m->blob + blob_floats, 0, (size_t)(total - blob_floats) * 4), "memset folded parameters");
        for (int l = 0; l < 3 && rc == SAPCU_OK && total > blob_floats; ++l) {
            const int d = 128 << l, sb = FN_BLK0 + l * B_SLOTS;
            const int64_t need[4] = {(int64_t)d * d, d, (int64_t)64 * d, 64};
            static const int slot[4] = {B_OUT_W, B_OUT_B, B_FC2_W, B_FC2_B};
            std::vector<float> h[4], wf((size_t)64 * d), bf(64);
            for (int q = 0; q < 4 && rc == SAPCU_OK; ++q) {
                if (m->dir[sb + slot[q]] + need[q] > blob_floats) {
                    set_error("model_create(fn): slot %d runs past the end of the blob", sb + slot[q]);
                    rc = SAPCU_ERR_ARG;
                    break;
                }
                h[q].resize((size_t)need[q]);
                hip_ok(hipMemcpy(h[q].data(), m->p(sb + slot[q]), (size_t)need[q] * 4, hipMemcpyDeviceToHost), "read out_proj / fc2");
            }
            if (rc != SAPCU_OK) break;
            fold_affine_f64(h[0].data(), h[1].data(), h[2].data(), h[3].data(), d, 64, wf.data(), bf.data());
            hip_ok(hipMemcpy(m->blob + m->fold_w[l], wf.data(), wf.size() * 4, hipMemcpyHostToDevice), "copy folded weights");
            if (rc == SAPCU_OK) hip_ok(hipMemcpy(m->blob + m->fold_b[l], bf.data(), bf.size() * 4, hipMemcpyHostToDevice), "copy folded bias");
        }
        if (rc == SAPCU_OK) hip_ok(hipMalloc((void**)&m->ovf_dev, 2 * sizeof(int)), "hipMalloc(ovf)");
        if (rc == SAPCU_OK) hip_ok(hipMemset(m->ovf_dev, 0, 2 * sizeof(int)), "memset ovf");
        if (rc == SAPCU_OK && m->sf16) {
            hip_ok(hipMalloc(&m->w16_hi, (size_t)total * 2), "hipMalloc(w16_hi)");
            if (rc == SAPCU_OK) hip_ok(hipMalloc(&m->w16_lo, (size_t)total * 2), "hipMalloc(w16_lo)");
            if (rc == SAPCU_OK) {
                int wovf = 0;
                if (launch_split_weights(m->blob, total, m->w16_hi, m->w16_lo, m->ovf_dev + 1, nullptr) != SAPCU_OK)
                    rc = SAPCU_ERR_HIP;
                if (rc == SAPCU_OK) hip_ok(hipMemcpy(&wovf, m->ovf_dev + 1, sizeof(int), hipMemcpyDeviceToHost), "read ovf");
                if (rc == SAPCU_OK && wovf != 0) m->sf16 = false;
            }
            if (rc == SAPCU_OK && m->sf16 && kind == SAPCU_KIND_FN) {
                hip_ok(hipMalloc(&m->chain_w, (size_t)chain_w_off(3, 0) * 2), "hipMalloc(chain_w)");
                for (int l = 0; l < 3 && rc == SAPCU_OK; ++l) {
                    const int d = 128 << l;
                    static const int slots[3] = {B_DELTA2_W, B_GAMMA_W, B_GAMMA2_W};
                    for (int q = 0; q < 3 && rc == SAPCU_OK; ++q) {
                        const int64_t wo = m->dir[FN_BLK0 + l * B_SLOTS + slots[q]];
                        if (launch_pack_chain_weights((const _Float16*)m->w16_hi + wo, (const _Float16*)m->w16_lo + wo, d,
                                                      (_Float16*)m->chain_w + chain_w_off(l, q), nullptr) != SAPCU_OK)
                            rc = SAPCU_ERR_HIP;
                    }
                }
                if (rc == SAPCU_OK) hip_ok(hipDeviceSynchronize(), "pack chain weights");
            }
        }
        if (rc == SAPCU_OK && kind == SAPCU_KIND_FD) {
            hip_ok(hipMalloc((void**)&m->ks_dev, 8 * sizeof(int32_t)), "hipMalloc(ks)");
            if (rc == SAPCU_OK) hip_ok(hipMemcpy(m->ks_dev, m->ks, 8 * sizeof(int32_t), hipMemcpyHostToDevice), "copy ks");
            if (rc == SAPCU_OK) hip_ok(hipMalloc((void**)&m->gate_dev, sizeof(int)), "hipMalloc(gate)");
            if (rc == SAPCU_OK) hip_ok(hipMemset(m->gate_dev, 0, sizeof(int)), "memset gate");
            if (rc == SAPCU_OK && m->sf16 && m->emb >= 96) {
                const int first = m->nscale <= 4 ? 0 : 4;
                const int mats[5][3] = {{FD_FUSE_W, 64, 64 * m->nscale}, {FD_EDGE1_W, 256, 64}, {FD_EDGE2_W, 512, 128},
                                        {FD_EDGE3_W, 1024, 256}, {FD_MSC_W, m->emb, 960}};
                int64_t halves = 0;
                for (int i = 0; i < 5; ++i) {
                    m->fde_off[i] = halves;
                    if (i >= first) halves += (int64_t)2 * mats[i][1] * mats[i][2];
                }
                hip_ok(hipMalloc(&m->fde_w, (size_t)halves * 2), "hipMalloc(fde_w)");
                if (rc == SAPCU_OK) hip_ok(hipMalloc((void**)&m->fde_nprm, 960 * 8 * sizeof(float)), "hipMalloc(fde_nprm)");
                for (int i = first; i < 5 && rc == SAPCU_OK; ++i) {
                    const int64_t wo = m->dir[mats[i][0]];
                    if (launch_pack_frag_weights((const _Float16*)m->w16_hi + wo, (const _Float16*)m->w16_lo + wo, mats[i][1], mats[i][2],
                                                 (_Float16*)m->fde_w + m->fde_off[i], nullptr) != SAPCU_OK)
                        rc = SAPCU_ERR_HIP;
                }
                static const int nslot[4] = {FD_SNN0, FD_SNN1, FD_SNN2, FD_SNN3}, nch[4] = {64, 128, 256, 512}, noff[4] = {0, 64, 192, 448};
                for (int i = 0; i < 4 && rc == SAPCU_OK; ++i)
                    if (launch_pack_fd_neuron(m->p(nslot[i]), nch[i], i < 2 ? 1 : 0, noff[i], m->fde_nprm, nullptr) != SAPCU_OK) rc = SAPCU_ERR_HIP;
                if (rc == SAPCU_OK) hip_ok(hipDeviceSynchronize(), "pack fd encoder operands");
            }
        }
    }
    if (rc != SAPCU_OK) {
        free_model(m);
        return rc;
    }
    *out = m;
    return SAPCU_OK;
}

int sapcu_internal_fold_affine_host(const float* w_out, const float* b_out, const float* w_fc2, const float* b_fc2, int d, int n,
                                    float* w_fold_out, float* b_fold_out) {
    SAPCU_CHECK_ARG(w_out && b_out && w_fc2 && b_fc2 && w_fold_out && b_fold_out && d >= 1 && n >= 1, "fold_affine: bad argument");
    fold_affine_f64(w_out, b_out, w_fc2, b_fc2, d, n, w_fold_out, b_fold_out);
    return SAPCU_OK;
}

int sapcu_model_destroy(sapcu_model_t m) {
    if (!m) return SAPCU_OK;
    free_model(m);
    return SAPCU_OK;
}

int64_t sapcu_workspace_bytes(sapcu_model_t m, int64_t b, int m_pts) {
    if (!m || b < 0 || m_pts < 1 || m_pts > 128) {
        set_error("workspace_bytes: bad argument");
        return SAPCU_ERR_ARG;
    }
    const size_t bytes = m->kind == SAPCU_KIND_FN ? fn_ws_layout(nullptr, m, fn_plan(m, b, m_pts), m_pts).bytes
                                                  : fd_ws_layout(nullptr, m, fd_plan(m, b, m_pts), m_pts).bytes;
    return (int64_t)bytes + 256;
}

int sapcu_model_gate_violations(sapcu_model_t m, int* count_host) {
    SAPCU_CHECK_ARG(m && count_host, "gate_violations: null pointer");
    *count_host = 0;
    if (m->gate_dev) SAPCU_CHECK_HIP(hipMemcpy(count_host, m->gate_dev, sizeof(int), hipMemcpyDeviceToHost));
    return SAPCU_OK;
}

int sapcu_model_gemm_mode(sapcu_model_t m, int* split_f16_host, int* range_overflows_host) {
    SAPCU_CHECK_ARG(m && split_f16_host && range_overflows_host, "gemm_mode: null pointer");
    *split_f16_host = m->sf16 ? 1 : 0;
    *range_overflows_host = 0;
    if (m->ovf_dev) SAPCU_CHECK_HIP(hipMemcpy(range_overflows_host, m->ovf_dev, sizeof(int), hipMemcpyDeviceToHost));
    return SAPCU_OK;
}

int sapcu_model_fused_blocks(sapcu_model_t m, int m_pts, int* mask_host) {
    SAPCU_CHECK_ARG(m && mask_host && m_pts >= 1 && m_pts <= 128, "fused_blocks: bad argument");
    int mask = 0;
    if (m->kind == SAPCU_KIND_FN) {
        for (int l = 0; l < 3; ++l)
            if (fn_block_fused(m, l, m_pts)) mask |= 1 << l;
    } else {
        if (fd_encoder_fused(m, m_pts)) mask = 1;
        else if (fd_x0_path(m, m_pts)) mask = 2;
    }
    *mask_host = mask;
    return SAPCU_OK;
}

int sapcu_fn_forward(sapcu_model_t m, const float* patch, int64_t b, int m_pts, const int32_t* knn_in, int32_t* knn_out,
                     float* normals_out, void* workspace, int64_t ws_bytes, void* const* taps_host, void* stream) {
    SAPCU_CHECK_ARG(m && m->kind == SAPCU_KIND_FN, "fn_forward: not an fn model handle");
    SAPCU_CHECK_ARG(patch && normals_out && workspace, "fn_forward: null pointer");
    SAPCU_CHECK_ARG(b >= 0 && m_pts >= 1 && m_pts <= 128, "fn_forward: need 1 <= m_pts <= 128 (got %d)", m_pts);
    return fn_forward(m, patch, b, m_pts, knn_in, knn_out, normals_out, workspace, ws_bytes, taps_host,
                      (hipStream_t)stream);
}

int sapcu_fd_forward(sapcu_model_t m, const float* patch, int64_t b, int m_pts, const int32_t* knn_force, float* dist_out,
                     void* workspace, int64_t ws_bytes, void* const* taps_host, void* stream) {
    SAPCU_CHECK_ARG(m && m->kind == SAPCU_KIND_FD, "fd_forward: not an fd model handle");
    SAPCU_CHECK_ARG(patch && dist_out && workspace, "fd_forward: null pointer");
    SAPCU_CHECK_ARG(b >= 0 && m_pts >= 1 && m_pts <= 128, "fd_forward: need 1 <= m_pts <= 128 (got %d)", m_pts);
    return fd_forward(m, patch, b, m_pts, knn_force, dist_out, workspace, ws_bytes, taps_host, (hipStream_t)stream);
}

}
```

### c-users-sayakdutta-self-supervised-arbitrary-scale-point-cloud-upsampling-via-snn_amd/csrc/ops.h

```cpp
#pragma once
#include "common.h"

namespace sapcu {

int launch_patch_knn_strided(const float* feat, int64_t b, int64_t pstride, int m, int c, int ld, int k,
                             int32_t* idx, hipStream_t st);
int launch_patch_knn_multi(const float* feat, int64_t b, int64_t pstride, int m, int c, int ld, int ntab,
                           const int* ks, int32_t* const* idx, hipStream_t st);
int launch_patch_knn(const float* feat, int64_t b, int m, int c, int ld, int k, int32_t* idx, hipStream_t st);
int launch_neuron_selfloop(const float* x, int64_t rows, int ch, int T, const float* md, const float* ta,
                           const float* rd, const float* tb, const float* dT, const float* rh, float* so, float* mo,
                           float* to, float* ro, hipStream_t st);
int launch_neuron_drive(const float* x, int64_t rows, int ch, int T, const float* md, const float* ta, const float* rd, const float* tb,
                        const float* dT, const float* rh, int pairv, float* so, float* mo, float* to, float* ro, int* gate, hipStream_t st);
int launch_fn_stem(const float* patch, int64_t rows, const float* w, const float* bias, const float* lif, int T,
                   float* out, hipStream_t st);
int launch_fn_pe1(const float* patch, const int32_t* idx, int64_t rows, int m, int kk, int d, const float* w,
                  const float* bias, const float* lif, int T, float* out, int split, hipStream_t st);
struct ChainArgs {
    int64_t P;
    int m;
    const int2* tab;
    const float4* pd;
    const float* qkv;
    int ldq;
    const float* wd;
    const float* bd;
    const float* lifd;
    const _Float16* w1p;
    const float* b1;
    const float* lif1;
    const _Float16* w2p;
    const float* b2;
    const float* lif2;
    const _Float16* w3p;
    const float* b3;
    float inv_sqrt_hd;
    float* res;
    int res_split;
    int T;
    int wide_offsets;
    float* fill_x;
    float* fill_t;
};
bool fn_edge_chain_ok(int d, int kk);
int launch_fn_edge_chain(ChainArgs a, const float* patch, const int32_t* idx, int d, int kk, int2* tab_ws, float4* pd_ws,
                         hipStream_t st);
int launch_pack_chain_weights(const void* w16_hi, const void* w16_lo, int d, void* out, hipStream_t st);
int launch_edge_table(const int32_t* idx, int64_t rows, int m, int kk, int2* tab, hipStream_t st);
int launch_fn_softmax_agg(const float* a, const float* pe, const float* v, int ldv, const int32_t* idx, int64_t pts,
                          int m, int kk, int d, float sqrt_hd, float* res, int split, hipStream_t st);
int launch_decode_max_keys(const unsigned* keys, int64_t count, float* out, hipStream_t st);
int launch_rowgroup_max(const float* in, int64_t groups, int m, int c, float* out, hipStream_t st);
int launch_fn_tail(const float* h, int64_t b, int kdim, const float* w, const float* bias, const float* lnw,
                   const float* lnb, float* logits, float* normals, hipStream_t st);
int launch_to_split_rows(const float* in, int64_t rows, int k, int ld_in, float* out, int ld_out, hipStream_t st);
int launch_l2_normalize3(const float* in, float* out, int64_t b, hipStream_t st);
int launch_fd_edge0(const float* patch, const int32_t* idx, int kmax, int64_t pts, int m, int nscale,
                    const int32_t* ks_dev, const float* w, const float* bias, float* out, hipStream_t st);
int launch_fd_neuron(bool eif, int mode, const float* in, int ldi, const int32_t* idx, int kk, int m,
                     const float* shift, int64_t pts, int C, const float* prm, int T, float* spk, int ldo, int coff,
                     float* pre_out, int* gate_violations, hipStream_t st, float* spk_split = nullptr,
                     float* x0_out = nullptr);
typedef _Float16 fe_half8 __attribute__((ext_vector_type(8)));
struct FdEncArgs {
    const float* patch;
    int64_t b;
    int64_t b_total, s0;
    int m, T, kk, kmax0, nscale, emb;
    int ks[4];
    const float* e0_w;
    const float* e0_b;
    const _Float16* fuse_wp;
    const float* fuse_b;
    const _Float16* edge_wp[3];
    const float* shift[3];
    const _Float16* msc_wp;
    const float* msc_b;
    const float* nprm;
    float* pooled;
    const int32_t* knn_force;
    int32_t* tap_knn;
    float* tap_fused0;
    float* tap_spikes;
    float* tap_x0;
    int* gate;
    int* ovf;
};
struct FdMscArgs {
    const float* x0;
    int64_t b;
    int64_t b_total, s0;
    int m, T, emb;
    const _Float16* msc_wp;
    const float* msc_b;
    const float* nprm;
    float* pooled;
    float* tap_spikes;
    int* gate;
};
bool fd_msc_ok(int m, int emb, int T);
int launch_fd_msc(const FdMscArgs& a, hipStream_t st);
bool fd_encoder_ok(int m, int nscale, int emb, int T);
int launch_fd_encoder(const FdEncArgs& a, hipStream_t st);
int launch_pack_frag_weights(const void* w16_hi, const void* w16_lo, int n, int k, void* out, hipStream_t st);
int launch_pack_fd_neuron(const float* raw, int C, int eif, int coff, float* out, hipStream_t st);
int launch_fd_pre(const float* in, int ldi, const int32_t* idx, int kk, int m, const float* shift, int64_t pts, int C, float* out,
                  int ldo, int coff, hipStream_t st);
int launch_fd_temporal(const float* pooled, int T, int64_t b, int emb, const float* tw, const float* lif, float* out,
                       hipStream_t st);
int launch_fd_tail(const float* x, const float* qkv, int64_t b, int heads, const float* wo_t, const float* bo,
                   const float* lnw, const float* lnb, const float* wh_t, const float* bh, const float* wd,
                   const float* bd, float* attn_out, float* dist, hipStream_t st);
int64_t train_column_sums_bytes(int64_t rows, int ch);
int train_column_sums(const float* a, int64_t rows, int ch, void* ws, double** sums_out, hipStream_t st);

}
```

Before: 131,600 query-points/s.

## Trim fn edge-chain epilogue: MFMA fc_delta and lane-shared spare-slot softmax

After: 133,100 query-points/s (median of 6 runs). +1.1%, better.

```diff
diff --git a/c-users-sayakdutta-self-supervised-arbitrary-scale-point-cloud-upsampling-via-snn_amd/csrc/fn_edge_chain.hip b/c-users-sayakdutta-self-supervised-arbitrary-scale-point-cloud-upsampling-via-snn_amd/csrc/fn_edge_chain.hip
--- a/c-users-sayakdutta-self-supervised-arbitrary-scale-point-cloud-upsampling-via-snn_amd/csrc/fn_edge_chain.hip
+++ b/c-users-sayakdutta-self-supervised-arbitrary-scale-point-cloud-upsampling-via-snn_amd/csrc/fn_edge_chain.hip
@@ -7,6 +7,9 @@
 
 #ifndef SAPCU_CHAIN_LB128
 #define SAPCU_CHAIN_LB128 3
+#endif
+#ifndef SAPCU_CHAIN_FCD_MFMA
+#define SAPCU_CHAIN_FCD_MFMA(D) ((D) == 256)
 #endif
 template <int D> struct ChainShape {
     static constexpr int ROWS = D == 128 ? 96 : (D == 256 ? 128 : 64);
@@ -75,6 +78,41 @@
     const auto q = __builtin_amdgcn_permlane32_swap(z, z, false, false);
     return __uint_as_float((s & 2) ? q[1] : q[0]);
 }
+
+__device__ __forceinline__ float lane_fetch(int byte_addr, float x) {
+    return __int_as_float(__builtin_amdgcn_ds_bpermute(byte_addr, __float_as_int(x)));
+}
+
+#ifdef CHAIN_STAMPS
+#define CHAIN_STAMP(IDX)                                                                                 \
+    do {                                                                                                 \
+        __builtin_amdgcn_sched_barrier(0);                                                               \
+        if (a.stamps && tid == 0) a.stamps[grp * 16 + (IDX)] = __builtin_amdgcn_s_memtime();             \
+        __builtin_amdgcn_sched_barrier(0);                                                               \
+    } while (0)
+#define CHAIN_T0() unsigned long long ch_t_own = 0, ch_t_spare = 0, ch_tp = __builtin_amdgcn_s_memtime()
+#define CHAIN_TACC(V)                                                          \
+    do {                                                                       \
+        __builtin_amdgcn_sched_barrier(0);                                     \
+        const unsigned long long now_ = __builtin_amdgcn_s_memtime();          \
+        ch_##V += now_ - ch_tp;                                                \
+        ch_tp = now_;                                                          \
+        __builtin_amdgcn_sched_barrier(0);                                     \
+    } while (0)
+#define CHAIN_STAMP_END()                                                      \
+    do {                                                                       \
+        if (a.stamps && tid == 0) {                                            \
+            a.stamps[grp * 16 + 13] = ch_t_own;                                \
+            a.stamps[grp * 16 + 14] = ch_t_spare;                              \
+            a.stamps[grp * 16 + 15] = __builtin_amdgcn_s_memtime();            \
+        }                                                                      \
+    } while (0)
+#else
+#define CHAIN_STAMP(IDX) do { } while (0)
+#define CHAIN_T0() do { } while (0)
+#define CHAIN_TACC(V) do { } while (0)
+#define CHAIN_STAMP_END() do { } while (0)
+#endif
 
 template <int CS>
 struct ChainLane {
@@ -234,7 +272,7 @@
 }
 
 template <int KK>
-__device__ __forceinline__ float chain_softmax_agg(float (&xs)[KK], const float (&ts)[KK]) {
+__device__ __forceinline__ float chain_softmax_den(float (&xs)[KK]) {
     float mx = -__builtin_huge_valf();
 #pragma unroll
     for (int jj = 0; jj < KK; ++jj) mx = fmaxf(mx, xs[jj]);
@@ -248,6 +286,11 @@
         den = __fadd_rn(den, xs[jj]);
         den = __fadd_rn(den, xs[jj + 1]);
     }
+    return den;
+}
+
+template <int KK>
+__device__ __forceinline__ float chain_softmax_out(const float (&xs)[KK], const float (&ts)[KK], float den) {
     const float inv_den = __fdiv_rn(1.0f, den);
     const f32x2 inv2 = f32x2{inv_den, inv_den};
     float out = 0.f;
@@ -260,14 +303,24 @@
     return out;
 }
 
-template <int D, int KK, bool O32, bool FILL>
+template <int KK>
+__device__ __forceinline__ float chain_softmax_agg(float (&xs)[KK], const float (&ts)[KK]) {
+    const float den = chain_softmax_den<KK>(xs);
+    return chain_softmax_out<KK>(xs, ts, den);
+}
+
+template <int D, int KK, bool O32, bool FILL, bool TRIM>
 __device__ __forceinline__ void fn_edge_chain_body(const ChainArgs& a) {
     static_assert(!FILL || (D == 512 && KK == 12), "filled groups: d = 512, kk = 12");
+    static_assert(ChainSlots<D, KK>::NUA == 0 || (ChainSlots<D, KK>::NUA == 1 && ChainSlots<D, KK>::SP == 4 && KK == 12) ||
+                      (ChainSlots<D, KK>::NUA == 3 && ChainSlots<D, KK>::SP == 14 && KK == 18),
+                  "the trimmed spare-slot sums are written for the slot layouts of d = 256 / kk = 18 and d = 512 / kk = 12");
     using S = ChainShape<D>;
     using M = ChainSlots<D, KK>;
     constexpr int CH_ROWS = S::ROWS, RS = S::RS, CS = S::CS, CH_PLANE = S::PLANE, CH_KSTEP = S::KSTEP;
     constexpr int PPG = M::PPG, NUA = M::NUA, SP = M::SP;
     constexpr int NUP = RS / 2;
+    constexpr bool TRIM_FCD = TRIM && SAPCU_CHAIN_FCD_MFMA(D);
     extern __shared__ __attribute__((aligned(1024))) unsigned char smem[];
     unsigned char* X = smem;
     float* pdx = reinterpret_cast<float*>(smem + CH_ROWS * D * 4);
@@ -316,6 +369,7 @@
 
     f32x4 acc[RS][CS], pe[RS][CS];
     ChainW<CS> W;
+    CHAIN_STAMP(0);
     if (tid < CH_ROWS) {
         const int rs = tid >> 4, sg = (tid >> 2) & 3, e = tid & 3, t = 4 * rs + e;
         int p, jj;
@@ -337,27 +391,55 @@
         pdx[tid] = dv.x;
         pdy[tid] = dv.y;
         pdz[tid] = dv.z;
-    }
+        if (TRIM_FCD) pdz[CH_ROWS + tid] = 1.0f;
+    }
+    CHAIN_STAMP(1);
     lds_barrier();
+    float pa[RS], wb[CS];
+    auto fc_delta_unit = [&](int j, int up) {
+#pragma unroll
+        for (int hq = 0; hq < 2; ++hq)
+            acc[2 * up + hq][j] = __builtin_amdgcn_mfma_f32_16x16x4f32(pa[2 * up + hq], wb[j], f32x4{-0.f, -0.f, -0.f, -0.f}, 0, 0, 0);
+    };
+    if (TRIM_FCD) {
+#pragma unroll
+        for (int i = 0; i < RS; ++i) pa[i] = pdx[L.g * CH_ROWS + 16 * i + L.c16];
+#pragma unroll
+        for (int j = 0; j < CS; ++j) wb[j] = L.g < 3 ? a.wd[L.col[j] * 3 + L.g] : a.bd[L.col[j]];
+        fc_delta_unit(0, 0);
+    }
 #pragma unroll
     for (int j = 0; j < CS; ++j) {
-        const float wx = a.wd[L.col[j] * 3], wy = a.wd[L.col[j] * 3 + 1], wz = a.wd[L.col[j] * 3 + 2], bd = a.bd[L.col[j]];
+        float wx = 0.f, wy = 0.f, wz = 0.f, bd = 0.f;
+        if (!TRIM_FCD) {
+            wx =a.wd[L.col[j] * 3];
+            wy = a.wd[L.col[j] * 3 + 1];
+            wz = a.wd[L.col[j] * 3 + 2];
+            bd = a.bd[L.col[j]];
+        }
         const NeuronP nd = chain_lif(a.lifd, D, L.col[j]);
 #pragma unroll
         for (int up = 0; up < NUP; ++up) {
             float v[8];
-#pragma unroll
-            for (int hq = 0; hq < 2; ++hq) {
-                const int r0 = 16 * (2 * up + hq) + rowg;
-                const float4 qx = *reinterpret_cast<const float4*>(pdx + r0), qy = *reinterpret_cast<const float4*>(pdy + r0),
-                             qz = *reinterpret_cast<const float4*>(pdz + r0);
-                const f32x2 wx2 = f32x2{wx, wx}, wy2 = f32x2{wy, wy}, wz2 = f32x2{wz, wz}, bd2 = f32x2{bd, bd};
-                const f32x2 ta = pk_fma(wz2, f32x2{qz.x, qz.y}, pk_fma(wy2, f32x2{qy.x, qy.y}, wx2 * f32x2{qx.x, qx.y})) + bd2;
-                const f32x2 tb = pk_fma(wz2, f32x2{qz.z, qz.w}, pk_fma(wy2, f32x2{qy.z, qy.w}, wx2 * f32x2{qx.z, qx.w})) + bd2;
-                v[4 * hq] = ta.x;
-                v[4 * hq + 1] = ta.y;
-                v[4 * hq + 2] = tb.x;
-                v[4 * hq + 3] = tb.y;
+            if (TRIM_FCD) {
+                if (up + 1 < NUP) fc_delta_unit(j, up + 1);
+                else if (j + 1 < CS) fc_delta_unit(j + 1, 0);
+#pragma unroll
+                for (int z = 0; z < 8; ++z) v[z] = acc[2 * up + (z >> 2)][j][z & 3];
+            } else {
+#pragma unroll
+                for (int hq = 0; hq < 2; ++hq) {
+                    const int r0 = 16 * (2 * up + hq) + rowg;
+                    const float4 qx = *reinterpret_cast<const float4*>(pdx + r0), qy = *reinterpret_cast<const float4*>(pdy + r0),
+                                 qz = *reinterpret_cast<const float4*>(pdz + r0);
+                    const f32x2 wx2 = f32x2{wx, wx}, wy2 = f32x2{wy, wy}, wz2 = f32x2{wz, wz}, bd2 = f32x2{bd, bd};
+                    const f32x2 ta = pk_fma(wz2, f32x2{qz.x, qz.y}, pk_fma(wy2, f32x2{qy.x, qy.y}, wx2 * f32x2{qx.x, qx.y})) + bd2;
+                    const f32x2 tb = pk_fma(wz2, f32x2{qz.z, qz.w}, pk_fma(wy2, f32x2{qy.z, qy.w}, wx2 * f32x2{qx.z, qx.w})) + bd2;
+                    v[4 * hq] = ta.x;
+                    v[4 * hq + 1] = ta.y;
+                    v[4 * hq + 2] = tb.x;
+                    v[4 * hq + 3] = tb.y;
+                }
             }
             lif_selfloop_n<8>(v, nd, a.T);
 #pragma unroll
@@ -365,6 +447,7 @@
             __builtin_amdgcn_sched_barrier(0);
         }
     }
+    CHAIN_STAMP(2);
     const half8* const wp1 = reinterpret_cast<const half8*>(a.w1p);
     const half8* const wp2 = reinterpret_cast<const half8*>(a.w2p);
     const half8* const wp3 = reinterpret_cast<const half8*>(a.w3p);
@@ -395,10 +478,13 @@
     gather_kv(0, 0, kq[0], vq[0]);
     chain_w_prefetch<D>(wp1, cs0, lane, W);
     lds_barrier();
+    CHAIN_STAMP(3);
 
     {
         chain_gemm<D>(X, wp1, cs0, lane, W, acc);
+        CHAIN_STAMP(4);
         lds_barrier();
+        CHAIN_STAMP(5);
 #pragma unroll
         for (int j = 0; j < CS; ++j) {
             const float b1 = a.b1[L.col[j]];
@@ -439,12 +525,16 @@
                 __builtin_amdgcn_sched_barrier(0);
             }
         }
+        CHAIN_STAMP(6);
         chain_w_prefetch<D>(wp2, cs0, lane, W);
     }
     lds_barrier();
+    CHAIN_STAMP(7);
     {
         chain_gemm<D>(X, wp2, cs0, lane, W, acc);
+        CHAIN_STAMP(8);
         lds_barrier();
+        CHAIN_STAMP(9);
 #pragma unroll
         for (int j = 0; j < CS; ++j) {
             const float b2 = a.b2[L.col[j]];
@@ -460,13 +550,16 @@
                 __builtin_amdgcn_sched_barrier(0);
             }
         }
+        CHAIN_STAMP(10);
         chain_w_prefetch<D>(wp3, cs0, lane, W);
     }
     lds_barrier();
+    CHAIN_STAMP(11);
     {
         chain_gemm<D>(X, wp3, cs0, lane, W, acc);
-#pragma unroll
-        for (int j = 0; j < CS; ++j) {
+        CHAIN_STAMP(12);
+        CHAIN_T0();
+        auto scale_rows = [&](int j) {
             const float b3 = a.b3[L.col[j]];
 #pragma unroll
             for (int i = 0; i < RS; ++i) {
@@ -485,53 +578,228 @@
                     }
                 }
             }
-            {
-                float xs[KK], ts[KK];
-#pragma unroll
-                for (int jj = 0; jj < KK; ++jj) {
-                    xs[jj] = acc[jj >> 2][j][jj & 3];
-                    ts[jj] = pe[jj >> 2][j][jj & 3];
-                }
-                const float out = chain_softmax_agg<KK>(xs, ts);
-                if (L.g < npts) {
-                    const int64_t pt = pt0 + L.g;
-                    if (a.res_split) chain_store_split_nt(a.res, pt, D, L.col[j], out);
-                    else __builtin_nontemporal_store(out, &a.res[pt * D + L.col[j]]);
-                }
-            }
-            if (NUA > 0) {
-                float xs[KK], ts[KK];
-#pragma unroll
-                for (int jj = 0; jj < KK; ++jj) {
-                    float cx[4] = {0.f, 0.f, 0.f, 0.f}, ct[4] = {0.f, 0.f, 0.f, 0.f};
-#pragma unroll
-                    for (int n = 0; n < NUA; ++n) {
-                        const int rs = M::ua_rs(n, jj), e = M::ua_e(n, jj), sg = M::ua_g(n, jj);
-                        cx[n] = group_bcast(acc[rs][j][e], sg);
-                        ct[n] = group_bcast(pe[rs][j][e], sg);
-                    }
-                    xs[jj] = NUA == 1 ? cx[0] : group_select(cx[0], cx[1], cx[2], cx[3], g0, g1);
-                    ts[jj] = NUA == 1 ? ct[0] : group_select(ct[0], ct[1], ct[2], ct[3], g0, g1);
-                }
-                const float out = chain_softmax_agg<KK>(xs, ts);
-                if (L.g < NUA && 4 + L.g < npts) {
-                    const int64_t pt = pt0 + 4 + L.g;
-                    if (a.res_split) chain_store_split_nt(a.res, pt, D, L.col[j], out);
-                    else __builtin_nontemporal_store(out, &a.res[pt * D + L.col[j]]);
-                }
-            }
-        }
-    }
-}
-
-template <int D, int KK, bool O32>
+        };
+        float own_den[CS];
+        auto own_first = [&](int j) {
+            float xs[KK];
+#pragma unroll
+            for (int jj = 0; jj < KK; ++jj) xs[jj] = acc[jj >> 2][j][jj & 3];
+            own_den[j] = chain_softmax_den<KK>(xs);
+#pragma unroll
+            for (int jj = 0; jj < KK; ++jj) acc[jj >> 2][j][jj & 3] = xs[jj];
+        };
+        auto own_second = [&](int j) {
+            float xs[KK], ts[KK];
+#pragma unroll
+            for (int jj = 0; jj < KK; ++jj) {
+                xs[jj] = acc[jj >> 2][j][jj & 3];
+                ts[jj] = pe[jj >> 2][j][jj & 3];
+            }
+            const float out = chain_softmax_out<KK>(xs, ts, own_den[j]);
+            if (L.g < npts) {
+                const int64_t pt = pt0 + L.g;
+                if (a.res_split) chain_store_split_nt(a.res, pt, D, L.col[j], out);
+                else __builtin_nontemporal_store(out, &a.res[pt * D + L.col[j]]);
+            }
+        };
+        if constexpr (!(NUA > 0 && TRIM)) {
+#pragma unroll
+            for (int j = 0; j < CS; ++j) {
+                scale_rows(j);
+                own_first(j);
+                own_second(j);
+                CHAIN_TACC(t_own);
+                if (NUA > 0) {
+                    float xs[KK], ts[KK];
+#pragma unroll
+                    for (int jj = 0; jj < KK; ++jj) {
+                        float cx[4] = {0.f, 0.f, 0.f, 0.f}, ct[4] = {0.f, 0.f, 0.f, 0.f};
+#pragma unroll
+                        for (int n = 0; n < NUA; ++n) {
+                            const int rs = M::ua_rs(n, jj), e = M::ua_e(n, jj), sg = M::ua_g(n, jj);
+                            cx[n] = group_bcast(acc[rs][j][e], sg);
+                            ct[n] = group_bcast(pe[rs][j][e], sg);
+                        }
+                        xs[jj] = NUA == 1 ? cx[0] : group_select(cx[0], cx[1], cx[2], cx[3], g0, g1);
+                        ts[jj] = NUA == 1 ? ct[0] : group_select(ct[0], ct[1], ct[2], ct[3], g0, g1);
+                    }
+                    const float out = chain_softmax_agg<KK>(xs, ts);
+                    if (L.g < NUA && 4 + L.g < npts) {
+                        const int64_t pt = pt0 + 4 + L.g;
+                        if (a.res_split) chain_store_split_nt(a.res, pt, D, L.col[j], out);
+                        else __builtin_nontemporal_store(out, &a.res[pt * D + L.col[j]]);
+                    }
+                }
+                CHAIN_TACC(t_spare);
+            }
+        } else {
+#define CHAIN_SX(J, S) acc[(KK + (S)) >> 2][J][(KK + (S)) & 3]
+#define CHAIN_ST(J, S) pe[(KK + (S)) >> 2][J][(KK + (S)) & 3]
+#pragma unroll
+            for (int j = 0; j < CS; ++j) scale_rows(j);
+            const int a_prev = ((lane + 48) & 63) * 4, a_next = ((lane + 16) & 63) * 4;
+            const float NEG = -__builtin_huge_valf();
+            const f32x2 l2e = f32x2{1.4426950408889634074f, 1.4426950408889634074f};
+            constexpr int NST = NUA == 3 ? 5 : 7, NH = 2 * CS;
+            float o_end[CS], u0[CS], u1[CS], u2[CS], u3[CS];
+            const bool fin[3] = {L.g > 0, L.g > 1, L.g > 2};
+            auto finishes = [&](int q) { return q < 3 && fin[q < 3 ? q : 0]; };
+            auto starts = [&](int q) { return q < 3 ? !fin[q] : !fin[2]; };
+            auto stage256 = [&](int k, int j) {
+                float(&mF)[CS] = u0, (&mS)[CS] = u1, (&rS)[CS] = u2, (&rF)[CS] = u3;
+                float(&dF)[CS] = u1, (&iS)[CS] = u2;
+                if (k == 0) {
+                    float f = NEG, s0 = NEG;
+#pragma unroll
+                    for (int q = 0; q < 4; ++q) {
+                        float mq = CHAIN_SX(j, 4 * q);
+#pragma unroll
+                        for (int s = 4 * q + 1; s < 4 * q + 4 && s < SP; ++s) mq = fmaxf(mq, CHAIN_SX(j, s));
+                        if (q < 3) f = finishes(q) ? fmaxf(f, mq) : f;
+                        s0 = starts(q) ? fmaxf(s0, mq) : s0;
+                    }
+                    mF[j] = f;
+                    mS[j] = s0;
+                    rS[j] = lane_fetch(a_prev, s0);
+                    rF[j] = lane_fetch(a_next, f);
+                } else if (k == 1) {
+                    const float xF = fmaxf(mF[j], rS[j]), xS = fmaxf(mS[j], rF[j]);
+#pragma unroll
+                    for (int s = 0; s < SP; s += 2) {
+                        const float mx = finishes(s >> 2) ? xF : xS;
+                        const f32x2 e2 = (f32x2{CHAIN_SX(j, s), CHAIN_SX(j, s + 1)} - f32x2{mx, mx}) * l2e;
+                        CHAIN_SX(j, s) = __builtin_amdgcn_exp2f(e2.x);
+                        CHAIN_SX(j, s + 1) = __builtin_amdgcn_exp2f(e2.y);
+                    }
+                    float d = 0.f;
+#pragma unroll
+                    for (int q = 0; q < 4; ++q) {
+                        float t = d;
+#pragma unroll
+                        for (int s = 4 * q; s < 4 * q + 4 && s < SP; ++s) t = __fadd_rn(t, CHAIN_SX(j, s));
+                        d = starts(q) ? t : d;
+                    }
+                    dF[j] = lane_fetch(a_prev, d);
+                } else if (k == 2) {
+                    float d = dF[j];
+#pragma unroll
+                    for (int q = 0; q < 3; ++q) {
+                        float t = d;
+#pragma unroll
+                        for (int s = 4 * q; s < 4 * q + 4; ++s) t = __fadd_rn(t, CHAIN_SX(j, s));
+                        d = finishes(q) ? t : d;
+                    }
+                    dF[j] = __fdiv_rn(1.0f, d);
+                    iS[j] = lane_fetch(a_next, dF[j]);
+                } else if (k == 3) {
+#pragma unroll
+                    for (int s = 0; s < SP; s += 2) {
+                        const float iv = finishes(s >> 2) ? dF[j] : iS[j];
+                        const f32x2 w2 = f32x2{CHAIN_SX(j, s), CHAIN_SX(j, s + 1)} * f32x2{iv, iv};
+                        CHAIN_SX(j, s) = w2.x;
+                        CHAIN_SX(j, s + 1) = w2.y;
+                    }
+                    float o = 0.f;
+#pragma unroll
+                    for (int q = 0; q < 4; ++q) {
+                        float t = o;
+#pragma unroll
+                        for (int s = 4 * q; s < 4 * q + 4 && s < SP; ++s) t = __fmaf_rn(CHAIN_SX(j, s), CHAIN_ST(j, s), t);
+                        o = starts(q) ? t : o;
+                    }
+                    o_end[j] = lane_fetch(a_prev, o);
+                } else {
+                    float o = o_end[j];
+#pragma unroll
+                    for (int q = 0; q < 3; ++q) {
+                        float t = o;
+#pragma unroll
+                        for (int s = 4 * q; s < 4 * q + 4; ++s) t = __fmaf_rn(CHAIN_SX(j, s), CHAIN_ST(j, s), t);
+                        o = finishes(q) ? t : o;
+                    }
+                    o_end[j] = o;
+                }
+            };
+            const int a_g0 = L.c16 * 4, a_g1 = (16 + L.c16) * 4, a_g2 = (32 + L.c16) * 4;
+            auto stage512 = [&](int k, int j) {
+                if (k == 0) {
+                    const float m = fmaxf(fmaxf(CHAIN_SX(j, 0), CHAIN_SX(j, 1)), fmaxf(CHAIN_SX(j, 2), CHAIN_SX(j, 3)));
+                    u0[j] = lane_fetch(a_g0, m);
+                    u1[j] = lane_fetch(a_g1, m);
+                    u2[j] = lane_fetch(a_g2, m);
+                } else if (k == 1 || k == 2 || k == 3) {
+                    if (k == 1) {
+                        const float mx = fmaxf(fmaxf(u0[j], u1[j]), u2[j]);
+#pragma unroll
+                        for (int s = 0; s < 4; s += 2) {
+                            const f32x2 e2 = (f32x2{CHAIN_SX(j, s), CHAIN_SX(j, s + 1)} - f32x2{mx, mx}) * l2e;
+                            CHAIN_SX(j, s) = __builtin_amdgcn_exp2f(e2.x);
+                            CHAIN_SX(j, s + 1) = __builtin_amdgcn_exp2f(e2.y);
+                        }
+                    }
+                    float t = k == 1 ? 0.f : u0[j];
+#pragma unroll
+                    for (int s = 0; s < 4; ++s) t = __fadd_rn(t, CHAIN_SX(j, s));
+                    if (k < 3) u0[j] = lane_fetch(a_prev, t);
+                    else u0[j] = lane_fetch(a_g2, __fdiv_rn(1.0f, t));
+                } else {
+                    if (k == 4) {
+#pragma unroll
+                        for (int s = 0; s < 4; s += 2) {
+                            const f32x2 w2 = f32x2{CHAIN_SX(j, s), CHAIN_SX(j, s + 1)} * f32x2{u0[j], u0[j]};
+                            CHAIN_SX(j, s) = w2.x;
+                            CHAIN_SX(j, s + 1) = w2.y;
+                        }
+                    }
+                    float t = k == 4 ? 0.f : u1[j];
+#pragma unroll
+                    for (int s = 0; s < 4; ++s) t = __fmaf_rn(CHAIN_SX(j, s), CHAIN_ST(j, s), t);
+                    o_end[j] = t;
+                    if (k < 6) u1[j] = lane_fetch(a_prev, t);
+                }
+            };
+#pragma unroll
+            for (int i = 0; i < (NST > NH ? NST : NH); ++i) {
+                if (i < NST) {
+#pragma unroll
+                    for (int j = 0; j < CS; ++j) {
+                        if constexpr (NUA == 3) stage256(i, j);
+                        else stage512(i, j);
+                    }
+                }
+                CHAIN_TACC(t_spare);
+                __builtin_amdgcn_sched_barrier(0);
+                if (i < NH) {
+                    if (i & 1) own_second(i >> 1);
+                    else own_first(i >> 1);
+                }
+                CHAIN_TACC(t_own);
+                __builtin_amdgcn_sched_barrier(0);
+            }
+            const int st_pt = NUA == 3 ? 3 + L.g : 4;
+            if ((NUA == 3 ? L.g > 0 : L.g == 2) && st_pt < npts) {
+#pragma unroll
+                for (int j = 0; j < CS; ++j) {
+                    if (a.res_split) chain_store_split_nt(a.res, pt0 + st_pt, D, L.col[j], o_end[j]);
+                    else __builtin_nontemporal_store(o_end[j], &a.res[(pt0 + st_pt) * D + L.col[j]]);
+                }
+            }
+            CHAIN_TACC(t_spare);
+#undef CHAIN_SX
+#undef CHAIN_ST
+        }
+        CHAIN_STAMP_END();
+    }
+}
+
+template <int D, int KK, bool O32, bool TRIM>
 __global__ __launch_bounds__(ChainShape<D>::NW * 64, (D == 128 ? SAPCU_CHAIN_LB128 : 1)) void fn_edge_chain_kernel(const ChainArgs a) {
-    fn_edge_chain_body<D, KK, O32, false>(a);
-}
-
-template <bool O32>
+    fn_edge_chain_body<D, KK, O32, false, TRIM>(a);
+}
+
+template <bool O32, bool TRIM>
 __global__ __launch_bounds__(ChainShape<512>::NW * 64, 1) void fn_edge_chain_fill_kernel(const ChainArgs a) {
-    fn_edge_chain_body<512, 12, O32, true>(a);
+    fn_edge_chain_body<512, 12, O32, true, TRIM>(a);
 }
 
 template <int KK>
@@ -553,30 +821,36 @@
     else __builtin_nontemporal_store(out, &res[pt * d + col]);
 }
 
-template <int D, int KK, bool O32>
+template <int D, int KK, bool O32, bool TRIM>
 static int launch_chain_t(const ChainArgs& a, hipStream_t st) {
     constexpr int lds = ChainShape<D>::LDS;
     static DeviceOnce lds_once;
-    SAPCU_SET_MAX_LDS(lds_once, (&fn_edge_chain_kernel<D, KK, O32>), lds);
+    SAPCU_SET_MAX_LDS(lds_once, (&fn_edge_chain_kernel<D, KK, O32, TRIM>), lds);
     constexpr int PPG = ChainSlots<D, KK>::PPG;
     const int64_t ngroups = (a.P + PPG - 1) / PPG;
     const int64_t grid = ngroups < 8 ? ngroups : ((ngroups + 7) / 8) * 8;
     SAPCU_CHECK_ARG(grid < 0x7fffffffLL, "edge_chain: too many groups");
-    hipLaunchKernelGGL((fn_edge_chain_kernel<D, KK, O32>), dim3((unsigned)grid), dim3(ChainShape<D>::NW * 64), lds, st, a);
+    hipLaunchKernelGGL((fn_edge_chain_kernel<D, KK, O32, TRIM>), dim3((unsigned)grid), dim3(ChainShape<D>::NW * 64), lds, st, a);
     SAPCU_CHECK_LAUNCH();
     return SAPCU_OK;
 }
 
-template <bool O32>
+template <int D, int KK>
+static int launch_chain_plain(const ChainArgs& a, bool o32, hipStream_t st) {
+    if (a.trim) return o32 ? launch_chain_t<D, KK, true, true>(a, st) : launch_chain_t<D, KK, false, true>(a, st);
+    return o32 ? launch_chain_t<D, KK, true, false>(a, st) : launch_chain_t<D, KK, false, false>(a, st);
+}
+
+template <bool O32, bool TRIM>
 static int launch_chain_fill_t(const ChainArgs& a, hipStream_t st) {
     constexpr int lds = ChainShape<512>::LDS, PPG = ChainSlots<512, 12>::PPG;
     static DeviceOnce lds_once;
-    SAPCU_SET_MAX_LDS(lds_once, (&fn_edge_chain_fill_kernel<O32>), lds);
+    SAPCU_SET_MAX_LDS(lds_once, (&fn_edge_chain_fill_kernel<O32, TRIM>), lds);
     const int64_t nsuper = a.P / 16;
     const int64_t ngroups = 3 * nsuper + (a.P - 16 * nsuper + PPG - 1) / PPG;
     const int64_t grid = ngroups < 8 ? ngroups : ((ngroups + 7) / 8) * 8;
     SAPCU_CHECK_ARG(grid < 0x7fffffffLL, "edge_chain: too many groups");
-    hipLaunchKernelGGL((fn_edge_chain_fill_kernel<O32>), dim3((unsigned)grid), dim3(ChainShape<512>::NW * 64), lds, st, a);
+    hipLaunchKernelGGL((fn_edge_chain_fill_kernel<O32, TRIM>), dim3((unsigned)grid), dim3(ChainShape<512>::NW * 64), lds, st, a);
     SAPCU_CHECK_LAUNCH();
     hipLaunchKernelGGL((fn_chain_straddler_kernel<12>), dim3((unsigned)((nsuper * 512 + 255) / 256)), dim3(256), 0, st, a.fill_x, a.fill_t,
                        nsuper, 512, a.res, a.res_split);
@@ -597,10 +871,13 @@
     a.tab = tab;
     a.pd = pd;
     const bool o32 = !a.wide_offsets && (uint64_t)a.P * (uint64_t)a.ldq * 4u + 3u * (uint64_t)d * 4u < (1ull << 32) && a.ldq > 0;
-    if (d == 128) return o32 ? launch_chain_t<128, 24, true>(a, st) : launch_chain_t<128, 24, false>(a, st);
-    if (d == 256) return o32 ? launch_chain_t<256, 18, true>(a, st) : launch_chain_t<256, 18, false>(a, st);
-    if (a.fill_x && a.fill_t && a.P >= 16) return o32 ? launch_chain_fill_t<true>(a, st) : launch_chain_fill_t<false>(a, st);
-    return o32 ? launch_chain_t<512, 12, true>(a, st) : launch_chain_t<512, 12, false>(a, st);
+    if (d == 128) return launch_chain_plain<128, 24>(a, o32, st);
+    if (d == 256) return launch_chain_plain<256, 18>(a, o32, st);
+    if (a.fill_x && a.fill_t && a.P >= 16) {
+        if (a.trim) return o32 ? launch_chain_fill_t<true, true>(a, st) : launch_chain_fill_t<false, true>(a, st);
+        return o32 ? launch_chain_fill_t<true, false>(a, st) : launch_chain_fill_t<false, false>(a, st);
+    }
+    return launch_chain_plain<512, 12>(a, o32, st);
 }
 
 int launch_pack_chain_weights(const void* w16_hi, const void* w16_lo, int d, void* out, hipStream_t st) {
diff --git a/c-users-sayakdutta-self-supervised-arbitrary-scale-point-cloud-upsampling-via-snn_amd/csrc/model.hip b/c-users-sayakdutta-self-supervised-arbitrary-scale-point-cloud-upsampling-via-snn_amd/csrc/model.hip
--- a/c-users-sayakdutta-self-supervised-arbitrary-scale-point-cloud-upsampling-via-snn_amd/csrc/model.hip
+++ b/c-users-sayakdutta-self-supervised-arbitrary-scale-point-cloud-upsampling-via-snn_amd/csrc/model.hip
@@ -79,6 +79,7 @@
     bool opt_chain = true;
     bool opt_chain_wide = false;
     bool opt_chain_fill = true;
+    bool opt_chain_trim = true;
     bool opt_shortk = true;
     bool opt_fn_maxfuse = true;
     bool opt_fn_fold_out = true;
@@ -136,6 +137,7 @@
     m->opt_chain = !env_is("SAPCU_CHAIN", "0");
     m->opt_chain_wide = env_is("SAPCU_CHAIN", "wide");
     m->opt_chain_fill = !env_is("SAPCU_CHAIN_FILL", "0");
+    m->opt_chain_trim = !env_is("SAPCU_CHAIN_TRIM", "0");
     m->opt_shortk = !env_is("SAPCU_SHORTK", "0");
     m->opt_fn_maxfuse = !env_is("SAPCU_FN_MAXFUSE", "0");
     m->opt_fn_fold_out = !env_is("SAPCU_FN_FOLD_OUT", "0");
@@ -324,6 +326,7 @@
     ca.w3p = cw + chain_w_off(e.l, 2); ca.b3 = m->p(sb + B_GAMMA2_B);
     ca.inv_sqrt_hd = 1.0f / e.sqrt_hd;
     ca.res = W.RES; ca.res_split = e.SP; ca.T = 4; ca.wide_offsets = m->opt_chain_wide ? 1 : 0;
+    ca.trim = m->opt_chain_trim ? 1 : 0;
     if (m->opt_chain_fill && d == 512 && e.kk == 12) {
         const int64_t need = (e.P / 16) * 12 * 512;
         if (need > 0 && need <= e.P * 512 && need <= e.b1_floats) {
@@ -923,6 +926,15 @@
     ca.w3p = W.packed[2]; ca.b3 = b3;
     ca.inv_sqrt_hd = 1.0f / (float)sqrt((double)(d / heads));
     ca.res = res_out; ca.res_split = 0; ca.T = lif_steps;
+    ca.trim = 1;
+#ifdef CHAIN_STAMPS
+    {
+        const int64_t sbytes = (points / 4 + 1) * 16 * 8;
+        const int64_t off = (need + 255) / 256 * 256;
+        if (workspace_bytes >= off + sbytes + 256) ca.stamps = (unsigned long long*)((char*)ws_align256(workspace) + off);
+        if (env_is("SAPCU_CHAIN_TRIM", "0")) ca.trim = 0;
+    }
+#endif
     return launch_fn_edge_chain(ca, patch, idx, d, kk, W.tab, W.pd, st);
 }
 
diff --git a/c-users-sayakdutta-self-supervised-arbitrary-scale-point-cloud-upsampling-via-snn_amd/csrc/ops.h b/c-users-sayakdutta-self-supervised-arbitrary-scale-point-cloud-upsampling-via-snn_amd/csrc/ops.h
--- a/c-users-sayakdutta-self-supervised-arbitrary-scale-point-cloud-upsampling-via-snn_amd/csrc/ops.h
+++ b/c-users-sayakdutta-self-supervised-arbitrary-scale-point-cloud-upsampling-via-snn_amd/csrc/ops.h
@@ -42,6 +42,10 @@
     int wide_offsets;
     float* fill_x;
     float* fill_t;
+    int trim;
+#ifdef CHAIN_STAMPS
+    unsigned long long* stamps;
+#endif
 };
 bool fn_edge_chain_ok(int d, int kk);
 int launch_fn_edge_chain(ChainArgs a, const float* patch, const int32_t* idx, int d, int kk, int2* tab_ws, float4* pd_ws,
diff --git a/profiles/chain_stamps.py b/profiles/chain_stamps.py
--- /dev/null
+++ b/profiles/chain_stamps.py
@@ -0,0 +1,66 @@
+#!/usr/bin/env python3
+import os
+import sys
+
+import numpy as np
+import torch
+
+sys.path.insert(0, os.path.dirname(os.path.dirname(os.path.abspath(__file__))))
+from sapcu_amd import _lib
+
+if os.environ.get("SAPCU_AB_LIB"):
+    _lib.LIB_PATH = os.environ["SAPCU_AB_LIB"]
+
+PPG = {128: 4, 256: 7, 512: 5}
+SPANS = [("phase 0: edge records", 0, 1), ("phase 0: fc_delta + neurons", 1, 2), ("(barrier)", 2, 3), ("GEMM 1", 3, 4),
+         ("(barrier)", 4, 5), ("epilogue 1", 5, 6), ("(barrier)", 6, 7), ("GEMM 2", 7, 8), ("(barrier)", 8, 9), ("epilogue 2", 9, 10),
+         ("(barrier)", 10, 11), ("GEMM 3", 11, 12), ("epilogue 3", 12, 15)]
+
+
+def main():
+    lib = _lib.load()
+    dev = torch.device("cuda")
+    B, M, heads, T = 4096, 48, 8, 4
+    P = B * M
+    print("lib %s, SAPCU_CHAIN_TRIM=%s; s_memtime ticks per group, median over the groups of one launch"
+          % (os.environ.get("SAPCU_AB_LIB", "default"), os.environ.get("SAPCU_CHAIN_TRIM", "(unset)")))
+    for d, kk in ((128, 24), (256, 18), (512, 12)):
+        g = torch.Generator(device="cpu").manual_seed(0)
+        patch = (torch.randn((B, M, 3), generator=g) * 0.05).to(dev)
+        idx = torch.stack([torch.randperm(M, generator=g)[:kk] for _ in range(P)]).to(torch.int32).to(dev)
+        qkv = torch.rand((P, 3 * d), generator=g).to(dev)
+
+        def lin(n, k, gain):
+            return ((torch.rand((n, k), generator=g) * 2 - 1) * gain / k ** 0.5).to(dev), (torch.randn(n, generator=g) * 0.4 + 0.6).to(dev)
+
+        def lif():
+            return torch.stack([torch.full((d,), 0.9), torch.full((d,), 0.01), torch.full((d,), 0.5), torch.ones(d)]).to(dev)
+
+        wd, bd = lin(d, 3, 20.0)
+        (w1, b1), (w2, b2), (w3, b3) = lin(d, d, 2.0), lin(d, d, 2.0), lin(d, d, 4.0)
+        ops = [patch.view(P, 3), idx.view(-1), qkv, wd, bd, lif(), w1, b1, lif(), w2, b2, lif(), w3, b3]
+        need = lib.sapcu_fn_edge_chain_workspace_bytes(P, d, kk)
+        off = (need + 255) // 256 * 256
+        sbytes = (P // 4 + 1) * 16 * 8
+        ws = torch.zeros(off + sbytes + 512, dtype=torch.uint8, device=dev)
+        res = torch.empty((P, d), device=dev)
+        for _ in range(2):
+            _lib.check(lib.sapcu_fn_edge_chain_f32(_lib.ptr(ops[0]), _lib.ptr(ops[1]), P, M, d, kk, *[_lib.ptr(t) for t in ops[2:]],
+                                                   heads, T, _lib.ptr(res), _lib.ptr(ws), ws.numel(), _lib.current_stream()))
+        torch.cuda.synchronize()
+        base = (-ws.data_ptr()) % 256
+        ngroups = (P + PPG[d] - 1) // PPG[d]
+        s = ws[base + off: base + off + ngroups * 128].cpu().numpy().view(np.int64).reshape(ngroups, 16).astype(np.float64)
+        if not s[:, 15].any():
+            print("d = %d: no stamps (not a -DCHAIN_STAMPS build?)" % d)
+            continue
+        total = np.median(s[:, 15] - s[:, 0])
+        print("d = %d, kk = %d: %d groups, total %.0f ticks per group, result sum %.6f" % (d, kk, ngroups, total, float(res.double().sum())))
+        for name, i0, i1 in SPANS:
+            v = np.median(s[:, i1] - s[:, i0])
+            print("  %-30s %8.0f  (%4.1f %%)" % (name, v, 100 * v / total))
+        print("  %-30s %8.0f   own points\n  %-30s %8.0f   points in spare slots" % ("  of epilogue 3:", np.median(s[:, 13]), "", np.median(s[:, 14])))
+
+
+if __name__ == "__main__":
+    main()
```
